# KMASAHIRO/AVR

Hardware: AMD Instinct MI355X
Metric: ray-samples/sec/GPU (1024 rays×256 samp×512 freq) + IR render ms/pose (higher is better)
Workload: dtype f32; 1 GPU; c2_meshrir_1024x256x512; mode=pose, rays=1024, samples=256, T=1022, freq_bins=512, distinct_poses=16, parallelism=poses x1 (no data-path collective)

## Files before the change

avr_amd/_lib.py:

```python
from __future__ import annotations

import ctypes
import math
import os
import threading

import numpy as np
import torch

_HERE = os.path.dirname(os.path.abspath(__file__))
LIB_PATH = os.path.join(_HERE, "libavr_hip.so")

DTYPE_F32 = 0
DTYPE_F16 = 1
DTYPE_BF16 = 2
MAX_AZI = 512
IRFFT_MAX_N = 13476

_c_i32 = ctypes.c_int32
_c_i64 = ctypes.c_int64
_c_f32 = ctypes.c_float
_vp = ctypes.c_void_p


# ... 19 lines not shown
        ("pl_len", _c_i32),
    ]

    def key(self):
        k = self.__dict__.get("_key")
        if k is None:
            k = self._key = tuple(getattr(self, f) for f, _ in self._fields_)
        return k


def _f32(x) -> float:
    return float(np.float32(x))


def render_params(cfg: dict, T: int, n_rays: int | None = None) -> RenderParams:
    p = RenderParams()
    p.n_azi = int(cfg["n_azi"])
    p.n_ele = int(cfg["n_ele"])
    p.n_samples = int(cfg["n_samples"])
    p.T = int(T)
    p.n_rays = p.n_azi * p.n_ele + 2 if n_rays is None else int(n_rays)
    p.depth_scale = _f32(cfg["far"] - cfg["near"])
    p.depth_offset = _f32(cfg["near"])
    p.lo = _f32(cfg["xyz_min"])
    p.span = _f32(cfg["xyz_max"] - cfg["xyz_min"])
    p.fs = _f32(cfg["fs"])
    p.speed = _f32(cfg["speed"])
    p.pathloss = _f32(cfg["pathloss"])
    p.azi_jitter = _f32(np.pi * 2 / cfg["n_azi"])
    p.two_pi = _f32(np.pi * 2)
    p.phase_c = _f32((-2 * np.pi) / T)
    p.near_clamp = int(0.1 / cfg["speed"] * cfg["fs"])
    p.pl_len = int(math.ceil(T * 2.5))
    return p


class TablePtrs(ctypes.Structure):

    _fields_ = [("d_vals", ctypes.c_void_p), ("shift", ctypes.c_void_p),
                ("pl_table", ctypes.c_void_p), ("phase", ctypes.c_void_p),
                ("twiddle", ctypes.c_void_p), ("ir_twiddle", ctypes.c_void_p)]


_SIGS = {
    "avr_last_error": (ctypes.c_char_p, []),
    "avr_abi_version": (ctypes.c_int, []),
    "avr_pinned_alloc": (ctypes.c_int, [_c_i64, _vp, _vp]),
    "avr_pinned_free": (ctypes.c_int, [_vp]),
    "avr_graph_launch": (ctypes.c_int, [_vp, _vp]),
    "avr_tables": (ctypes.c_int, [_vp, _vp, _vp, _vp, _vp, _vp, _vp, _vp]),
    "avr_depth_samples": (ctypes.c_int, [_vp, _vp, _vp]),
    "avr_ir_twiddle": (ctypes.c_int, [_c_i32, _vp, _vp]),
    "avr_ray_directions": (ctypes.c_int, [_vp, _vp, _vp, _vp]),
    "avr_sample_points": (ctypes.c_int, [_vp, _c_i32] + [_vp] * 10),
    "avr_sample_rays": (ctypes.c_int, [_vp, _c_i32, _vp, _c_i32] + [_vp] * 9),
    "avr_weights_fwd": (ctypes.c_int, [_vp, _c_i32, _vp, _c_i32] + [_vp] * 7),
    "avr_ray_reduce_fwd": (ctypes.c_int, [_vp, _c_i32, _vp, _c_i32, _vp, _vp, _c_i32, _vp, _vp]),
    "avr_sample_rays_dev": (ctypes.c_int, [_vp, _c_i32, _vp, _c_i32] + [_vp] * 9),
    "avr_sample_rays_staged": (ctypes.c_int, [_vp, _c_i32, _vp, _c_i32, _c_i32] + [_vp] * 7),
    "avr_reduce_splits": (ctypes.c_int, [_vp, _c_i32, _c_i32, _vp]),
    "avr_ray_reduce_mc_fwd": (ctypes.c_int, [_vp, _c_i32, _c_i32, _vp, _c_i32, _vp, _vp, _vp, _c_i64, _c_i32,
                                             _vp, _vp]),
    "avr_reduce_mc_splits": (ctypes.c_int, [_vp, _c_i32, _c_i32, _c_i32, _vp, _vp]),
    "avr_ray_reduce_mc16_fwd": (ctypes.c_int, [_vp, _c_i32, _c_i32, _vp, _c_i32, _vp, _vp, _vp, _c_i64, _c_i32,
                                               _vp, _vp]),
    "avr_reduce_mc16_max_rays": (_c_i32, []),
    "avr_sh_decode_fwd": (ctypes.c_int, [_c_i32, _c_i32, _c_i32, _c_i32, _vp, _vp, _vp, _vp]),
    "avr_sh_decode_bwd": (ctypes.c_int, [_c_i32, _c_i32, _c_i32, _c_i32, _vp, _vp, _vp, _vp]),
    "avr_ray_reduce_mc_bwd": (ctypes.c_int, [_vp, _c_i32, _c_i32, _vp, _c_i32, _vp, _vp, _vp, _vp, _c_i64,
                                             _vp, _vp, _vp]),
    "avr_dft_phase_fwd": (ctypes.c_int, [_vp, _c_i32, _vp, _c_i32, _vp, _vp, _vp, _vp, _c_i32, _vp, _vp]),
    "avr_spectrum_finalize": (ctypes.c_int, [_c_i32, _c_i32, _c_i32, _vp, _vp, _vp]),
    "avr_irfft": (ctypes.c_int, [_c_i32, _c_i32, _vp, _vp, _vp, _vp]),
    "avr_irfft_bwd": (ctypes.c_int, [_c_i32, _c_i32, _vp, _vp, _vp, _vp]),
    "avr_dft_phase_bwd": (ctypes.c_int, [_vp, _c_i32] + [_vp] * 7),
    "avr_ray_reduce_bwd": (ctypes.c_int, [_vp, _c_i32, _vp, _c_i32] + [_vp] * 6),
    "avr_weights_bwd": (ctypes.c_int, [_vp, _c_i32, _vp, _c_i32, _vp, _vp, _vp, _vp]),
    "avr_hashgrid_fwd": (ctypes.c_int, [_c_i64, _c_i32, _vp, _vp, _c_i32, _vp, _vp, _vp, _vp, _c_i32, _vp]),
    "avr_hashgrid_fwd_lm": (ctypes.c_int, [_c_i64, _c_i32, _vp, _vp, _c_i32, _vp, _vp, _vp, _vp, _c_i32, _vp]),
    "avr_hashgrid_fwd_lm_unit": (ctypes.c_int, [_c_i64, _c_i32, _vp, _vp, _c_i32, _vp, _vp, _vp, _vp, _c_i32, _vp]),
    "avr_ray_pose_bias": (ctypes.c_int, [_c_i32, _c_i32, _c_i32, _vp, _vp, _c_i32, _vp, _vp, _vp, _vp,
                                         _c_i32, _vp, _vp, _vp, _vp, _c_i32, _c_i32, _c_i32, _vp, _vp,
                                         _c_i32, _vp, _vp]),
    "avr_hashgrid_bwd": (ctypes.c_int, [_c_i64, _c_i32, _vp, _vp, _c_i32, _vp, _vp, _vp, _vp, _vp]),
    "avr_hashgrid_bwd_workspace": (ctypes.c_int, [_c_i64, _c_i32, _vp, _vp]),
    "avr_hashgrid_bwd_partitioned": (ctypes.c_int, [_c_i64, _c_i32, _vp, _vp, _c_i32, _vp, _vp, _vp, _vp, _vp,
                                                    _c_i64, _vp]),
    "avr_hashgrid_bwd_partitioned_set": (ctypes.c_int, [_c_i64, _c_i32, _vp, _vp, _c_i32, _vp, _vp, _vp, _vp, _vp,
                                                    _c_i64, _vp]),
    "avr_hashgrid_bwd_input_workspace": (ctypes.c_int, [_c_i64, _c_i32, _vp]),
    "avr_hashgrid_bwd_input": (ctypes.c_int, [_c_i64, _c_i32, _vp, _vp, _c_i32, _vp, _c_i32, _vp, _vp, _vp, _vp, _vp,
                                              _c_i64, _vp]),
    "avr_linear_wgrad_splits": (ctypes.c_int, [_c_i64, _c_i32, _c_i32, _vp]),
    "avr_linear512_pack_w2": (ctypes.c_int, [_vp, _c_i32, _c_i32, _vp, _vp]),
    "avr_linear512_mask_fwd": (ctypes.c_int, [_c_i64, _vp, _vp, _c_i32, _vp, _vp, _vp]),
    "avr_linear_wgrad": (ctypes.c_int, [_c_i64, _c_i32, _c_i32, _vp, _vp, _vp, _c_i32, _vp, _vp]),
    "avr_linear_out1_fwd": (ctypes.c_int, [_c_i64, _c_i32, _vp, _vp, _c_i32, _vp, _vp]),
    "avr_narrow_mm": (ctypes.c_int, [_c_i64, _c_i32, _c_i32, _vp, _vp, _c_i32, _c_i32, _vp, _vp, _vp]),
    "avr_linear_out1_workspace": (ctypes.c_int, [_c_i32, _vp]),
    "avr_linear_out1_bwd": (ctypes.c_int, [_c_i64, _c_i32, _vp, _vp, _vp, _c_i32, _vp, _vp, _vp, _vp]),
    "avr_head_splits": (ctypes.c_int, [_vp, _c_i32, _c_i32, _c_i32, _vp]),
    "avr_head_sort": (ctypes.c_int, [_vp, _c_i32, _vp, _vp, _vp, _vp, _vp, _vp]),
    "avr_head_pack_w": (ctypes.c_int, [_vp, _c_i32, _c_i32, _vp, _c_i32, _vp, _vp]),
    "avr_head_exact_layout": (ctypes.c_int, [_vp, _c_i32, _c_i32, _c_i32, _vp, _vp]),
    "avr_head_pack_w_exact": (ctypes.c_int, [_vp, _c_i32, _vp, _c_i32, _vp, _vp]),
    "avr_head_fwd_exact": (ctypes.c_int, [_vp, _c_i32, _c_i32, _vp, _vp, _c_i32, _vp, _vp, _vp, _vp, _c_i32,
                                          _vp, _vp, _vp]),
    "avr_head_fwd": (ctypes.c_int, [_vp, _c_i32, _c_i32, _vp, _vp, _c_i32, _vp, _vp, _vp, _c_i32, _vp,
                                    _vp]),
    "avr_head_bwd_workspace": (ctypes.c_int, [_vp, _c_i32, _c_i32, _c_i32, _vp]),
    "avr_head_bwd": (ctypes.c_int, [_vp, _c_i32, _c_i32, _vp, _vp, _c_i32, _vp, _vp, _vp, _vp, _vp, _vp,
                                    _vp, _vp, _vp, _vp, _c_i64, _vp]),
    "avr_head_bwd2": (ctypes.c_int, [_vp, _c_i32, _c_i32, _vp, _vp, _c_i32, _vp, _vp, _vp, _vp, _vp, _vp,
                                     _c_i32, _vp, _vp, _vp, _vp, _c_i64, _vp]),
    "avr_criterion_window_len": (ctypes.c_int, []),
    "avr_criterion_workspace": (ctypes.c_int, [_c_i32, _c_i32, _vp]),
    "avr_criterion_fwd": (ctypes.c_int, [_c_i32, _c_i32] + [_vp] * 10 + [_c_i64, _vp]),
    "avr_criterion_fwd2": (ctypes.c_int, [_c_i32, _c_i32] + [_vp] * 11 + [_c_i64, _vp]),
    "avr_criterion_bwd": (ctypes.c_int, [_c_i32, _c_i32] + [_vp] * 11 + [_c_i64, _vp, _vp]),
    "avr_das_workspace": (ctypes.c_int, [_vp]),
    "avr_das_fwd": (ctypes.c_int, [_c_i32] + [_vp] * 5 + [_c_f32] * 3 + [_vp, _vp, _c_i64, _vp]),
    "avr_das_bwd": (ctypes.c_int, [_c_i32] + [_vp] * 3 + [_c_f32] * 3 + [_vp, _vp, _c_i64, _vp, _vp]),
    "avr_metrics_workspace": (ctypes.c_int, [_c_i32, _c_i32, _vp]),
    "avr_metrics": (ctypes.c_int, [_c_i32, _c_i32, ctypes.c_double, _c_i32, _c_i32] + [_vp] * 10
                    + [_c_i64, _vp]),
    "avr_scale_sanitize": (ctypes.c_int, [_c_i32, _vp, _vp, _vp, _vp]),
    "avr_grad_clip_workspace": (ctypes.c_int, [_c_i32, _vp, _vp]),
    "avr_grad_clip_coef": (ctypes.c_int, [_c_i32, _vp, _vp, ctypes.c_float, _vp, ctypes.c_int64, _vp, _vp, _vp]),
    "avr_adam_step": (ctypes.c_int, [_c_i32, _vp, _vp, _vp, _vp, _vp, _vp, _vp, ctypes.c_double, ctypes.c_double,
                                     ctypes.c_float, ctypes.c_float, _vp, _vp]),
    "avr_concat_fwd": (ctypes.c_int, [_c_i64, _c_i32, _vp, _vp, _c_i32, _vp]),
    "avr_concat_bwd": (ctypes.c_int, [_c_i64, _c_i32, _vp, _vp, _c_i32, _vp, _vp]),
    "avr_group_bias_relu_fwd": (ctypes.c_int, [_c_i64, _c_i32, _c_i64, _c_i32, _vp, _c_i32, _vp, _vp, _vp, _vp]),
    "avr_group_bias_relu_workspace": (ctypes.c_int, [_c_i64, _c_i32, _c_i64, _vp]),
    "avr_group_bias_relu_bwd": (ctypes.c_int, [_c_i64, _c_i32, _c_i64, _c_i32, _vp, _vp, _c_i32, _vp, _vp, _vp,
                                               _c_i64, _vp, _vp]),
    "avr_conv_source": (ctypes.c_int, [_c_i32, _c_i32, _c_i32, _c_i64, _vp, _vp, _vp, _vp]),
    "avr_conv_trajectory": (ctypes.c_int, [_c_i32, _c_i32, _c_i32, _c_i64, _c_i64, _c_i64, _vp, _vp, _vp, _vp]),
    "avr_sosfiltfilt_workspace": (ctypes.c_int, [_c_i64, _c_i64, _c_i32, _c_i32, _vp]),
    "avr_sosfiltfilt": (ctypes.c_int, [_c_i64, _c_i64, _c_i32, _c_i32, _vp, _vp, _vp, _c_i32, _vp, _c_i32,
                                       _vp, _c_i64, _vp]),
    "avr_doa_das_workspace": (ctypes.c_int, [_c_i64, _c_i32, _c_i32, _vp]),
    "avr_doa_das": (ctypes.c_int, [_c_i64, _c_i32, _c_i32, _c_i32, _vp, _vp, _vp, _vp, _vp, ctypes.c_double,
                                   _vp, _vp, _c_i32, _vp, _vp, _c_i64, _vp]),
    "avr_doa_frames": (ctypes.c_int, [_c_i64, _c_i64, _c_i32, _c_i32, _c_i64, _c_i32, _c_i32, _c_i32, _c_i32,
                                      _c_i32, _c_f32, _vp, _c_i32, _vp, _vp, _vp, _vp, _vp, _vp, _vp]),
    "avr_doa_frame_stats": (ctypes.c_int, [_c_i64, _c_i64, _vp, _vp, _vp, _vp, _vp, _vp]),
    "avr_sigma_pack_bytes": (ctypes.c_int, [_c_i32, _vp]),
    "avr_sigma_desc_size": (ctypes.c_int, []),
    "avr_sigma_fwd": (ctypes.c_int, [_vp] * 3 + [_c_i32, _vp, _vp]),
    "avr_render_core_layout": (ctypes.c_int, [_vp, _c_i32, _c_i32, _vp, _vp]),
    "avr_render_core_fwd": (ctypes.c_int, [_vp, _c_i32, _vp, _c_i32, _vp, _c_i32] + [_vp] * 5
                            + [_c_i64] + [_vp] * 5),
}

EXPORTS = tuple(_SIGS)

_SHAPES_SIGS = {
    "avr_linear512_pack_w": (ctypes.c_int, [_vp, _c_i32, _vp, _vp]),
    "avr_linear512_relu_fwd": (ctypes.c_int, [_c_i64, _vp, _vp, _c_i32, _vp, _vp]),
    "avr_mlp512x2_pack_w": (ctypes.c_int, [_vp, _vp, _c_i32, _vp, _vp]),
    "avr_mlp512x2_fwd": (ctypes.c_int, [_c_i64, _vp, _vp, _c_i32, _vp, _vp]),
    "avr_linear_pack_w": (ctypes.c_int, [_c_i32, _c_i32, _vp, _c_i32, _vp, _vp]),
}

_lock = threading.Lock()
_lib = None


def load():
    global _lib
    if _lib is not None:
        return _lib
    with _lock:
        if _lib is not None:
            return _lib
        if not os.path.exists(LIB_PATH):
            raise RuntimeError(
                f"avr_amd: HIP library not found at {LIB_PATH}; build it with "
                "`python -c 'import __graft_entry__ as g; g.build()'` (make -C avr_amd/csrc)")
        lib = ctypes.CDLL(LIB_PATH)
        for name, (res, args) in _SIGS.items():
            fn = getattr(lib, name)
            fn.restype = res
            fn.argtypes = args
        for name, (res, args) in _SHAPES_SIGS.items():
            if hasattr(lib, name):
                fn = getattr(lib, name)
                fn.restype = res
                fn.argtypes = args
# ... 21 lines not shown
```

avr_amd/csrc/common.h:

```cpp
#pragma once

#include <hip/hip_runtime.h>
#include <hip/hip_fp16.h>
#include <hip/hip_bf16.h>
#include <type_traits>
#include <stdint.h>
#include <string>
#include <utility>

#include "avr_hip.h"

namespace avr {

void set_error(const std::string& msg);
int fail(int code, const std::string& msg);
int check_launch(const char* what);
int device_cus();

#define AVR_REQUIRE(cond, msg)                          \
    do {                                                \
        if (!(cond)) return ::avr::fail(AVR_E_ARG, msg); \
    } while (0)

int validate_render_params(const avr_render_params* p);

int launch_irfft(int B, int F, const float* spec, const float* spec2, const float* tw, float* ir,
                 float* ir2, void* stream);
constexpr int kIrfftMaxN = AVR_IRFFT_MAX_N;
constexpr size_t kLdsPerCu = 160 * 1024;
#define AVR_IRFFT_LIMIT_TEXT "irfft length n > 13476 not supported (n*12 B of twiddles and data must fit the 160 KiB LDS)"

int mr3_workspace(int B, int n, int64_t* bytes);
int launch_mr3(int B, int n, const float* pred_time, const float* ori_time, const float* wtab,
               const float* tw512, void* ws, int64_t ws_bytes, float* out, void* stream);

inline hipStream_t as_stream(void* s) { return reinterpret_cast<hipStream_t>(s); }

constexpr size_t kLdsDefault = 64 * 1024;

template <typename Kern, typename... Args>
int launch(const char* what, Kern kern, dim3 grid, dim3 block, size_t lds, hipStream_t st,
           Args&&... args) {
    if (lds > kLdsPerCu)
        return fail(AVR_E_CONFIG, std::string(what) + ": " + std::to_string(lds) +
                                      " B of dynamic LDS exceed a CU's 160 KiB");
    if (lds > kLdsDefault) {
        const hipError_t e = hipFuncSetAttribute((const void*)kern,
                                                 hipFuncAttributeMaxDynamicSharedMemorySize, (int)lds);
        if (e != hipSuccess)
            return fail((int)e, std::string(what) + ": LDS opt-in: " + hipGetErrorString(e));
    }
    hipLaunchKernelGGL(kern, grid, block, lds, st, std::forward<Args>(args)...);
    return check_launch(what);
}

constexpr int64_t align_up(int64_t x, int64_t a) { return (x + a - 1) & ~(a - 1); }

class Arena {
  public:
    Arena(void* base, int64_t align) : base_(static_cast<char*>(base)), align_(align) {}
    template <typename T>
    T* take(int64_t count) {
        char* r = base_ ? base_ + off_ : nullptr;
        off_ += align_up(count * (int64_t)sizeof(T), align_);
        return reinterpret_cast<T*>(r);
    }
    int64_t offset() const { return off_; }
    int64_t bytes() const { return off_; }

  private:
    char* base_;
    int64_t align_, off_ = 0;
};

template <int Code>
struct dtype_tag;
template <>
struct dtype_tag<AVR_DTYPE_F32> { using type = float; };
template <>
struct dtype_tag<AVR_DTYPE_F16> { using type = __half; };
template <>
struct dtype_tag<AVR_DTYPE_BF16> { using type = __hip_bfloat16; };

template <int... Allowed, typename F>
int dispatch_dtype(int code, const char* what, F&& f) {
    int rc = 0;
    const bool hit = ((code == Allowed ? (rc = f(dtype_tag<Allowed>{}), true) : false) || ...);
    return hit ? rc : fail(AVR_E_ARG, std::string(what) + ": unsupported dtype");
}

__device__ __forceinline__ void mfma_queue_wait() {
    __builtin_amdgcn_sched_barrier(0);
    asm volatile("s_nop 7");
}
template <typename T>
__device__ __forceinline__ void keep_live(const T& v) {
    asm volatile("" ::"v"(v));
}

__device__ __forceinline__ float load_f(const float* p, int64_t i) { return p[i]; }
__device__ __forceinline__ float load_f(const __half* p, int64_t i) { return __half2float(p[i]); }
__device__ __forceinline__ float load_f(const __hip_bfloat16* p, int64_t i) {
    return __bfloat162float(p[i]);
}
__device__ __forceinline__ void store_f(float* p, int64_t i, float v) { p[i] = v; }
__device__ __forceinline__ void store_f(__half* p, int64_t i, float v) { p[i] = __float2half(v); }
__device__ __forceinline__ void store_f(__hip_bfloat16* p, int64_t i, float v) {
    p[i] = __float2bfloat16(v);
}
__device__ __forceinline__ float bf16_lo(uint32_t u) { return __uint_as_float(u << 16); }
__device__ __forceinline__ float bf16_hi(uint32_t u) { return __uint_as_float(u & 0xffff0000u); }
__device__ __forceinline__ float f16_lo(uint32_t u) { return __half2float(__ushort_as_half((unsigned short)(u & 0xffffu))); }
__device__ __forceinline__ float f16_hi(uint32_t u) { return __half2float(__ushort_as_half((unsigned short)(u >> 16))); }

template <typename T>
__device__ __forceinline__ float unpack16(uint32_t u, int hi) {
    if constexpr (std::is_same<T, __half>::value)
        return hi ? f16_hi(u) : f16_lo(u);
    else
// ... 167 lines not shown
```

avr_amd/csrc/hashgrid.hip:

```cpp
#include "common.h"

#include <algorithm>

using namespace avr;

namespace {

constexpr int kMaxLevels = 32;

struct LevelTable {
    int64_t offset[kMaxLevels + 1];
    float scale[kMaxLevels];
    uint32_t res[kMaxLevels];
};

__device__ __forceinline__ uint32_t grid_index(uint32_t size, uint32_t res, uint32_t x, uint32_t y,
                                               uint32_t z) {
    uint64_t stride = 1;
    uint32_t index = 0;
    const uint32_t c[3] = {x, y, z};
#pragma unroll
    for (int d = 0; d < 3; ++d) {
        if (stride > size) break;
        index += c[d] * (uint32_t)stride;
// ... 101 lines not shown
            w *= 1.0f - c.pos[d];
            g[d] = c.grid[d];
        }
    }
    e = grid_index(size, res, g[0], g[1], g[2]);
}

__device__ __forceinline__ void corner_dx(const Corner& c, int k, uint32_t size, uint32_t res, float (&dw)[3],
                                          uint32_t& e) {
    float om[3];
    uint32_t g[3];
#pragma unroll
    for (int d = 0; d < 3; ++d) {
        const bool up = k & (1 << d);
        om[d] = up ? c.pos[d] : 1.0f - c.pos[d];
        g[d] = up ? c.grid[d] + 1 : c.grid[d];
    }
    const float w12 = om[1] * om[2], w02 = om[0] * om[2], w01 = om[0] * om[1];
    dw[0] = (k & 1) ? w12 : -w12;
    dw[1] = (k & 2) ? w02 : -w02;
    dw[2] = (k & 4) ? w01 : -w01;
    e = grid_index(size, res, g[0], g[1], g[2]);
}

template <typename Tp>
__device__ __forceinline__ float2 encode_point_level(const float* xi, const Level<const Tp>& lv) {
    const Corner c = locate(xi, lv.scale);
    CornerAcc<Tp> acc;
#pragma unroll
    for (int k = 0; k < 8; ++k) {
        float w;
        uint32_t e;
        corner(c, k, lv.size, lv.res, w, e);
        acc.add(w, CornerAcc<Tp>::load(lv.table, e));
    }
    return acc.get();
}

template <typename Tp, typename To>
__global__ __launch_bounds__(256) void hashgrid_fwd_kernel(int64_t N, int L,
                                                           const float* __restrict__ x,
                                                           const Tp* __restrict__ params,
                                                           LevelTable lt, To* __restrict__ out) {
    const int64_t q = (int64_t)blockIdx.x * blockDim.x + threadIdx.x;
    if (q >= N * L) return;
    const int64_t i = q / L;
    const int l = (int)(q % L);
    const float xi[3] = {x[i * 3 + 0], x[i * 3 + 1], x[i * 3 + 2]};
    const Level<const Tp> lv = level_view(lt, l, params);
    const Corner c = locate(xi, lv.scale);
    CornerAcc<Tp> acc;
#pragma unroll
    for (int k = 0; k < 8; ++k) {
        float w;
        uint32_t e;
        corner(c, k, lv.size, lv.res, w, e);
        acc.add(w, CornerAcc<Tp>::load(lv.table, e));
    }
    store_pair(out, q, acc.get());
}

template <typename Tp>
struct EntryGroup;
template <>
struct EntryGroup<__half> {
    static constexpr uint32_t kN = 4;
    uint32_t d[4];
    __device__ __forceinline__ void load(const __half* table, uint32_t e) {
        const uint4 v = *reinterpret_cast<const uint4*>(table + 2 * (e & ~(kN - 1)));
        d[0] = v.x;
        d[1] = v.y;
        d[2] = v.z;
        d[3] = v.w;
    }
    __device__ __forceinline__ __half2 get(uint32_t e) const {
        const uint32_t j = e & (kN - 1);
        const uint32_t v = j == 0 ? d[0] : j == 1 ? d[1] : j == 2 ? d[2] : d[3];
        __half2 h;
        __builtin_memcpy(&h, &v, 4);
        return h;
    }
};

template <typename Tp, typename To, bool ROW_MAJOR = false, bool GROUP = false>
__global__ __launch_bounds__(256) void hashgrid_fwd_lm_kernel(int64_t N, const float* __restrict__ x,
                                                              const Tp* __restrict__ params,
                                                              LevelTable lt, To* __restrict__ out, int unit) {
    const int l = blockIdx.y;
    const int64_t i = (int64_t)blockIdx.x * 256 + threadIdx.x;
    if (i >= N) return;
    float xi[3] = {x[i * 3 + 0], x[i * 3 + 1], x[i * 3 + 2]};
    if (unit) {
#pragma unroll
        for (int d = 0; d < 3; ++d) xi[d] = 0.5f + 0.5f * xi[d];
    }
    const Level<const Tp> lv = level_view(lt, l, params);
    const Tp* table = lv.table;
    const Corner c = locate(xi, lv.scale);
    CornerAcc<Tp> acc;
    float wgt[8];
    uint32_t ent[8];
#pragma unroll
    for (int k = 0; k < 8; ++k) corner(c, k, lv.size, lv.res, wgt[k], ent[k]);
    if constexpr (GROUP) {
        constexpr uint32_t kN = EntryGroup<Tp>::kN;
        EntryGroup<Tp> grp[4];
#pragma unroll
        for (int j = 0; j < 4; ++j) grp[j].load(table, ent[2 * j]);
        using raw = typename CornerAcc<Tp>::raw;
        raw far[4];
#pragma unroll
        for (int j = 0; j < 4; ++j) {
            far[j] = grp[j].get(ent[2 * j]);
            if ((ent[2 * j + 1] ^ ent[2 * j]) >= kN) far[j] = CornerAcc<Tp>::load(table, ent[2 * j + 1]);
        }
#pragma unroll
        for (int j = 0; j < 4; ++j) {
            const raw v0 = grp[j].get(ent[2 * j]);
            const raw v1 = ((ent[2 * j + 1] ^ ent[2 * j]) >= kN) ? far[j] : grp[j].get(ent[2 * j + 1]);
            acc.add(wgt[2 * j], v0);
            acc.add(wgt[2 * j + 1], v1);
        }
    } else {
#pragma unroll
        for (int k = 0; k < 8; ++k) acc.add(wgt[k], CornerAcc<Tp>::load(table, ent[k]));
    }
    store_pair(out, ROW_MAJOR ? i * (int64_t)gridDim.y + l : (int64_t)l * N + i, acc.get());
}

template <typename Tp, typename Tg>
__global__ __launch_bounds__(256) void hashgrid_dx_level_kernel(int64_t N, const float* __restrict__ x,
                                                                const Tp* __restrict__ params,
                                                                const Tg* __restrict__ gout, LevelTable lt,
                                                                float* __restrict__ partial) {
    const int l = blockIdx.y, L = gridDim.y;
    const int64_t i = (int64_t)blockIdx.x * 256 + threadIdx.x;
    if (i >= N) return;
    const float xi[3] = {x[i * 3 + 0], x[i * 3 + 1], x[i * 3 + 2]};
    const float g0 = load_f(gout, i * (2 * L) + 2 * l), g1 = load_f(gout, i * (2 * L) + 2 * l + 1);
    const Level<const Tp> lv = level_view(lt, l, params);
    const Corner c = locate(xi, lv.scale);
    float dw[8][3];
    uint32_t ent[8];
#pragma unroll
    for (int k = 0; k < 8; ++k) corner_dx(c, k, lv.size, lv.res, dw[k], ent[k]);
    float2 v[8];
#pragma unroll
    for (int k = 0; k < 8; ++k) v[k] = load_pair<Tp>(lv.table, ent[k]);
    float acc[3] = {0.0f, 0.0f, 0.0f};
#pragma unroll
    for (int k = 0; k < 8; ++k) {
        const float t = fmaf(g1, v[k].y, g0 * v[k].x);
#pragma unroll
        for (int d = 0; d < 3; ++d) acc[d] = fmaf(dw[k][d], t, acc[d]);
    }
    float* p = partial + ((int64_t)l * N + i) * 3;
#pragma unroll
    for (int d = 0; d < 3; ++d) p[d] = lv.scale * acc[d];
}

__global__ __launch_bounds__(256) void hashgrid_dx_sum_kernel(int64_t M, int L, const float* __restrict__ partial,
                                                              float* __restrict__ grad_x) {
    const int64_t j = (int64_t)blockIdx.x * 256 + threadIdx.x;
    if (j >= M) return;
    float s = 0.0f;
    for (int l = 0; l < L; ++l) s += partial[(int64_t)l * M + j];
    grad_x[j] = s;
}

template <typename Tg, int RUN>
__global__ __launch_bounds__(256) void hashgrid_bwd_kernel(int64_t N, int L, int l0,
                                                           const float* __restrict__ x,
                                                           const Tg* __restrict__ gout,
                                                           LevelTable lt,
                                                           float* __restrict__ gparams) {
    const int l = l0 + (int)blockIdx.y;
    const int slot = threadIdx.x & 15;
    const int k = slot >> 1, f = slot & 1;
    const int64_t first = ((int64_t)blockIdx.x * 16 + (threadIdx.x >> 4)) * RUN;
    const Level<float> lv = level_view(lt, l, gparams);
    float* __restrict__ table = lv.table;
    float xi[RUN][3], g[RUN];
#pragma unroll
    for (int it = 0; it < RUN; ++it) {
        const int64_t i = first + it;
        const int64_t ic = i < N ? i : N - 1;
#pragma unroll
        for (int d = 0; d < 3; ++d) xi[it][d] = x[ic * 3 + d];
        g[it] = i < N ? load_f(gout, ic * (2 * L) + 2 * l + f) : 0.0f;
    }
    uint32_t pe = 0xffffffffu;
    float pv = 0.0f;
#pragma unroll
    for (int it = 0; it < RUN; ++it) {
        float wgt;
        uint32_t ce;
        corner(locate(xi[it], lv.scale), k, lv.size, lv.res, wgt, ce);
        const uint32_t e = 2u * ce + (uint32_t)f;
        const float v = wgt * g[it];
        if (e == pe) {
            pv += v;
        } else {
            if (pv != 0.0f) atomicAdd(table + pe, pv);
            pe = e;
            pv = v;
        }
    }
    if (pv != 0.0f) atomicAdd(table + pe, pv);
}

// ... 580 lines not shown
                  0);
}

extern "C" int avr_hashgrid_fwd_lm_unit(int64_t N, int32_t n_levels, const float* x, const void* params,
                                        int32_t param_dtype, const int64_t* level_offset,
                                        const float* level_scale, const int32_t* level_res, void* out,
                                        int32_t out_dtype, void* stream) {
    return fwd_lm(N, n_levels, x, params, param_dtype, level_offset, level_scale, level_res, out, out_dtype, stream,
                  1);
}

namespace {

constexpr int kBiasRays = 4;

__device__ __forceinline__ float round_feature(float v, bool f16, bool mlp_f16) {
    if (f16) v = __half2float(__float2half(v));
    return mlp_f16 ? __half2float(__float2half(v))
                   : __bfloat162float(__float2bfloat16(v));
}

template <typename Tp>
__device__ __forceinline__ void bias_features(bool is_tx, int64_t b, int64_t r, int R, int S, const float* view,
                                              const float* tx, const Tp* dp, const LevelTable& dl, const Tp* tp,
                                              const LevelTable& tl, int l, int f16, int mlp_f16, float* e) {
    const float* src = is_tx ? tx + b * R * S * 3 : view + (b * R * S + r * S) * 3;
    const float xi[3] = {(src[0] + 1.0f) / 2.0f, (src[1] + 1.0f) / 2.0f, (src[2] + 1.0f) / 2.0f};
    const float2 v = is_tx ? encode_point_level(xi, level_view(tl, l, tp)) : encode_point_level(xi, level_view(dl, l, dp));
    e[2 * l] = round_feature(v.x, f16, mlp_f16);
    e[2 * l + 1] = round_feature(v.y, f16, mlp_f16);
}

template <typename Tp>
__global__ __launch_bounds__(256) void ray_pose_bias_kernel(int B, int R, int S, const float* __restrict__ view,
                                                            const float* __restrict__ tx, const Tp* __restrict__ dp,
                                                            LevelTable dl, int dL, const Tp* __restrict__ tp,
                                                            LevelTable tl, int tL, int f16, int mlp_f16,
                                                            const float* __restrict__ wd,
                                                            const float* __restrict__ wt, int nout,
                                                            float* __restrict__ bias) {
    __shared__ float e[kBiasRays][2][2 * kMaxLevels];
    const int64_t g0 = (int64_t)blockIdx.x * kBiasRays;
    const int nr = (int)min((int64_t)kBiasRays, (int64_t)B * R - g0);
    for (int q = threadIdx.x; q < kBiasRays * 2 * kMaxLevels; q += 256) {
        const int j = q / (2 * kMaxLevels), rem = q % (2 * kMaxLevels);
        const int which = rem / kMaxLevels, l = rem % kMaxLevels;
        if (j >= nr || l >= (which ? tL : dL)) continue;
        const int64_t gr = g0 + j;
        bias_features(which, gr / R, gr % R, R, S, view, tx, dp, dl, tp, tl, l, f16, mlp_f16, e[j][which]);
    }
    __syncthreads();
    auto skinny = [&](const float* __restrict__ w, int K2, int which, int o, float (&acc)[kBiasRays]) {
        int k = 0;
        for (; k + 8 <= K2; k += 8) {
            float wv[8];
#pragma unroll
            for (int u = 0; u < 8; ++u) wv[u] = w[(int64_t)(k + u) * nout + o];
#pragma unroll
            for (int u = 0; u < 8; ++u)
#pragma unroll
                for (int j = 0; j < kBiasRays; ++j) acc[j] = fmaf(e[j][which][k + u], wv[u], acc[j]);
        }
        for (; k < K2; ++k) {
            const float wv = w[(int64_t)k * nout + o];
#pragma unroll
            for (int j = 0; j < kBiasRays; ++j) acc[j] = fmaf(e[j][which][k], wv, acc[j]);
        }
    };
    for (int o = threadIdx.x; o < nout; o += 256) {
        float sd[kBiasRays], st[kBiasRays];
#pragma unroll
        for (int j = 0; j < kBiasRays; ++j) sd[j] = st[j] = 0.0f;
        skinny(wd, 2 * dL, 0, o, sd);
        skinny(wt, 2 * tL, 1, o, st);
#pragma unroll
        for (int j = 0; j < kBiasRays; ++j)
            if (j < nr) bias[(g0 + j) * nout + o] = sd[j] + st[j];
    }
}

constexpr int kBias2Rays = 4;
constexpr int kBias2Threads = 512;

template <typename Tp>
__global__ __launch_bounds__(kBias2Threads) void ray_pose_bias2_kernel(
    int B, int R, int S, const float* __restrict__ view, const float* __restrict__ tx, const Tp* __restrict__ dp,
    LevelTable dl, int dL, const Tp* __restrict__ tp, LevelTable tl, int tL, int f16, int mlp_f16,
    const float* __restrict__ wd, const float* __restrict__ wt, int nout, float* __restrict__ bias) {
    __shared__ float ed[kBias2Rays][2 * kMaxLevels];
    __shared__ float et[2 * kMaxLevels];
    const int64_t g0 = (int64_t)blockIdx.x * kBias2Rays;
    const int64_t b = g0 / R;
    for (int q = threadIdx.x; q < (kBias2Rays + 1) * kMaxLevels; q += kBias2Threads) {
        const int j = q / kMaxLevels, l = q % kMaxLevels;
        const bool is_tx = j == kBias2Rays;
        if (l >= (is_tx ? tL : dL)) continue;
        bias_features(is_tx, b, (g0 + j) % R, R, S, view, tx, dp, dl, tp, tl, l, f16, mlp_f16, is_tx ? et : ed[j]);
    }
    __syncthreads();
    for (int o = threadIdx.x; o < nout; o += kBias2Threads) {
        constexpr int KB = 16;
        float st = 0.0f;
        for (int k0 = 0; k0 < 2 * tL; k0 += KB) {
            float w[KB];
#pragma unroll
            for (int u = 0; u < KB; ++u) w[u] = k0 + u < 2 * tL ? wt[(int64_t)(k0 + u) * nout + o] : 0.0f;
#pragma unroll
            for (int u = 0; u < KB; ++u)
                if (k0 + u < 2 * tL) st = fmaf(et[k0 + u], w[u], st);
        }
        float sd[kBias2Rays];
#pragma unroll
        for (int r = 0; r < kBias2Rays; ++r) sd[r] = 0.0f;
        for (int k0 = 0; k0 < 2 * dL; k0 += KB) {
            float w[KB];
#pragma unroll
            for (int u = 0; u < KB; ++u) w[u] = k0 + u < 2 * dL ? wd[(int64_t)(k0 + u) * nout + o] : 0.0f;
#pragma unroll
            for (int u = 0; u < KB; ++u)
                if (k0 + u < 2 * dL)
#pragma unroll
                    for (int r = 0; r < kBias2Rays; ++r) sd[r] = fmaf(ed[r][k0 + u], w[u], sd[r]);
        }
#pragma unroll
        for (int r = 0; r < kBias2Rays; ++r) bias[(g0 + r) * nout + o] = sd[r] + st;
    }
}

}

extern "C" int avr_ray_pose_bias(int32_t B, int32_t R, int32_t S, const float* view, const float* tx,
                                 int32_t dir_levels, const void* dir_params, const int64_t* dir_offset,
                                 const float* dir_scale, const int32_t* dir_res, int32_t tx_levels,
                                 const void* tx_params, const int64_t* tx_offset, const float* tx_scale,
                                 const int32_t* tx_res, int32_t param_dtype, int32_t enc_dtype,
                                 int32_t mlp_dtype, const float* w_dir, const float* w_tx, int32_t n_out,
                                 float* bias, void* stream) {
    AVR_REQUIRE(B >= 1 && R >= 1 && S >= 1 && view && tx && dir_params && tx_params && w_dir && w_tx && bias &&
                    n_out >= 1,
                "avr_ray_pose_bias: bad args");
    AVR_REQUIRE(enc_dtype == AVR_DTYPE_F16 || enc_dtype == AVR_DTYPE_F32, "avr_ray_pose_bias: enc dtype");
    AVR_REQUIRE(mlp_dtype == AVR_DTYPE_BF16 || mlp_dtype == AVR_DTYPE_F16, "avr_ray_pose_bias: mlp dtype");
    const int mlp_f16 = mlp_dtype == AVR_DTYPE_F16;
    LevelTable dl, tl;
    if (int e = make_table(dir_levels, dir_offset, dir_scale, dir_res, &dl)) return e;
    if (int e = make_table(tx_levels, tx_offset, tx_scale, tx_res, &tl)) return e;
    const int64_t rays = (int64_t)B * R;
    const dim3 grid((unsigned)((rays + kBiasRays - 1) / kBiasRays));
    const int f16 = enc_dtype == AVR_DTYPE_F16;
    hipStream_t st = as_stream(stream);
    const bool v2 = R % kBias2Rays == 0;
    return dispatch_dtype<AVR_DTYPE_F16, AVR_DTYPE_F32>(param_dtype, "avr_ray_pose_bias", [&](auto tag) {
        using Tp = typename decltype(tag)::type;
        auto go = [&](auto kern, dim3 g, dim3 block) {
            return launch("avr_ray_pose_bias", kern, g, block, 0, st, (int)B, (int)R, (int)S, view, tx,
                          (const Tp*)dir_params, dl, (int)dir_levels, (const Tp*)tx_params, tl, (int)tx_levels, f16,
                          mlp_f16, w_dir, w_tx, (int)n_out, bias);
        };
        if (v2) return go(ray_pose_bias2_kernel<Tp>, dim3((unsigned)(rays / kBias2Rays)), dim3(kBias2Threads));
        return go(ray_pose_bias_kernel<Tp>, grid, dim3(256));
    });
}

constexpr int64_t kPartitionedMinPoints = 16384;

extern "C" int avr_hashgrid_bwd_workspace(int64_t N, int32_t n_levels, const int64_t* level_offset,
                                          int64_t* bytes) {
    AVR_REQUIRE(N >= 0 && level_offset && bytes, "avr_hashgrid_bwd_workspace: bad args");
    if (N < kPartitionedMinPoints) {
        *bytes = 256;
        return 0;
    }
    if (n_levels < 1 || n_levels > kMaxLevels) return fail(AVR_E_ARG, "hashgrid: n_levels out of range (1..32)");
    BwdLayout b;
    *bytes = (bwd_layout(N, n_levels, level_offset, nullptr, &b) == 0 && b.scatter_ok) ? b.bytes : 256;
    return 0;
}

namespace {
int bwd_partitioned(int64_t N, int32_t n_levels, const float* x, const void* grad_out, int32_t grad_dtype,
                    const int64_t* level_offset, const float* level_scale, const int32_t* level_res,
                    float* grad_params, void* workspace, int64_t workspace_bytes, void* stream, bool overwrite) {
    AVR_REQUIRE(N >= 0 && x && grad_out && level_offset && level_scale && level_res && grad_params && workspace,
                "avr_hashgrid_bwd_partitioned: bad args");
    AVR_REQUIRE(reinterpret_cast<uintptr_t>(grad_params) % 16 == 0 && reinterpret_cast<uintptr_t>(workspace) % 256 == 0,
                "avr_hashgrid_bwd_partitioned: grad_params must be 16-byte, workspace 256-byte aligned");
    AVR_REQUIRE(grad_dtype == AVR_DTYPE_F32 || grad_dtype == AVR_DTYPE_F16,
                "avr_hashgrid_bwd_partitioned: unknown grad dtype");
    LevelTable lt;
    if (int e = make_table(n_levels, level_offset, level_scale, level_res, &lt)) return e;
    hipStream_t st = as_stream(stream);
    const int L = n_levels;
    const char* what = "avr_hashgrid_bwd_partitioned";
    BwdLayout b;
    if (N < kPartitionedMinPoints || bwd_layout(N, n_levels, level_offset, level_res, &b) != 0 || !b.scatter_ok) {
        if (overwrite &&
            hipMemsetAsync(grad_params, 0, (size_t)(2 * level_offset[L]) * sizeof(float), st) != hipSuccess)
            return fail(AVR_E_ARG, "avr_hashgrid_bwd_partitioned_set: clear failed");
        return N == 0 ? 0 : launch_bwd(what, st, N, L, x, grad_out, grad_dtype, lt, grad_params);
    }
    AVR_REQUIRE(workspace_bytes >= b.bytes, "avr_hashgrid_bwd_partitioned: workspace too small");
    char* ws = static_cast<char*>(workspace);
    int* counts = reinterpret_cast<int*>(ws + b.counts);
    int* totals = reinterpret_cast<int*>(ws + b.totals);
    uint3* contrib = reinterpret_cast<uint3*>(ws + b.contrib);
    const dim3 grid((unsigned)b.plan.nchunks, (unsigned)L);
    const size_t lds_count = (size_t)b.plan.max_parts * 4;
    const size_t lds_scat = (size_t)(3 * kScatMaxRecs + 3 * b.plan.max_parts + 1) * 4;
    const dim3 tgrid((unsigned)((N + 63) / 64));
    void* glm = ws + b.glm;
    int* part_start = reinterpret_cast<int*>(ws + b.part_start);
    int* slice_base = reinterpret_cast<int*>(ws + b.slice_base);
    if (int e = dispatch_dtype<AVR_DTYPE_F32, AVR_DTYPE_F16>(grad_dtype, what, [&](auto tag) {
            using Tg = typename decltype(tag)::type;
            const Tg* g = (const Tg*)glm;
            if (int e = launch(what, hg_level_major_kernel<Tg>, tgrid, dim3(256), 64 * 2 * L * sizeof(Tg), st, N, L,
                               (const Tg*)grad_out, (Tg*)glm))
                return e;
            if (int e = launch(what, hg_bwd_count_kernel<Tg>, grid, dim3(256), lds_count, st, N, L, x, g, lt, b.plan,
                               counts))
                return e;
            if (int e = launch(what, hg_bwd_scan_kernel, dim3((unsigned)((b.total_parts + 15) / 16)), dim3(1024), 0,
                               st, b.total_parts, b.plan.nchunks, counts, totals))
                return e;
            if (int e = launch(what, hg_bwd_plan_kernel, dim3(1), dim3(1024), 0, st, b.total_parts, b.plan, totals,
                               part_start, slice_base))
                return e;
            return launch(what, hg_bwd_scatter_kernel<Tg>, grid, dim3(256), lds_scat, st, N, L, x, g, lt, b.plan,
                          counts, totals, part_start, contrib);
        }))
        return e;
    if (overwrite)
        if (int e = launch(what, hg_bwd_zero_hot_kernel, dim3((unsigned)b.total_parts), dim3(256), 0, st, lt, b.plan,
                           b.total_parts, slice_base, grad_params))
            return e;
    return launch(what, hg_bwd_reduce_kernel, dim3((unsigned)((b.max_slices + kReduceWaves - 1) / kReduceWaves)),
                  dim3(64 * kReduceWaves), 0, st, lt, b.plan, b.total_parts, totals, part_start, slice_base, contrib,
                  grad_params, (int)overwrite);
}
}

extern "C" int avr_hashgrid_bwd_partitioned(int64_t N, int32_t n_levels, const float* x, const void* grad_out,
                                            int32_t grad_dtype, const int64_t* level_offset,
// ... 56 lines not shown
```

avr_amd/csrc/head.hip:

```cpp
#include "common.h"

using namespace avr;

namespace {

constexpr int kThreads = 256;

__device__ __forceinline__ void lds_barrier() {
    __builtin_amdgcn_s_waitcnt(0xC07F);
    __builtin_amdgcn_s_barrier();
}

template <typename Th, int KB>
struct Raw {
    static constexpr int NB = KB * (int)sizeof(Th);
    static constexpr int ND = NB / 4;
    uint32_t d[ND];
    __device__ __forceinline__ void load(const Th* p) {
        if constexpr (NB % 16 == 0) {
#pragma unroll
            for (int c = 0; c < NB / 16; ++c) {
                const u32x4 v = reinterpret_cast<const u32x4*>(p)[c];
                d[4 * c] = v[0];
                d[4 * c + 1] = v[1];
// ... 320 lines not shown
        for (int k = 0; k < KB; ++k) run[k] = fmaf(wr[u], hv[u][k], run[k]);
    float off[KB];
#pragma unroll
    for (int k = 0; k < KB; ++k) {
        const float x = wave_scan_incl(run[k]);
        off[k] = dpp<0x138, 0xf, true>(x);
        if (lane == 63) wtotf[wave * KB + k] = x;
    }
    lds_barrier();
#pragma unroll
    for (int k = 0; k < KB; ++k) {
        float o = 0.0f;
        for (int w = 0; w < wave; ++w) o += wtotf[w * KB + k];
        off[k] += o;
    }
    if (threadIdx.x == 0)
#pragma unroll
        for (int k = 0; k < KB; ++k) C[k * RS + 3] = 0.0f;
    if (RPT % 4 == 0 && spt == RPT) {
        if (p0 < n)
#pragma unroll
            for (int k = 0; k < KB; ++k) {
                float r = 0.0f;
#pragma unroll
                for (int c = 0; c < RPT / 4; ++c) {
                    float v[4];
#pragma unroll
                    for (int e = 0; e < 4; ++e) {
                        r = fmaf(wr[4 * c + e], hv[4 * c + e][k], r);
                        v[e] = off[k] + r;
                    }
                    *reinterpret_cast<f32x4*>(C + k * RS + 4 + p0 + 4 * c) = f32x4{v[0], v[1], v[2], v[3]};
                }
            }
    } else {
#pragma unroll
        for (int k = 0; k < KB; ++k) {
            float r = 0.0f;
#pragma unroll
            for (int u = 0; u < RPT; ++u) {
                r = fmaf(wr[u], hv[u][k], r);
                if (u < spt && p0 + u < n) C[k * RS + 4 + p0 + u] = off[k] + r;
            }
        }
    }
}

template <int RPT>
struct Owned {
    int ray[RPT];
    float w[RPT];
    int n, spt;
    __device__ __forceinline__ void load(const int* __restrict__ perm, const float* __restrict__ ws,
                                         const int* __restrict__ cnt, int T) {
        n = cnt[T - 1];
        spt = (n + kThreads - 1) / kThreads;
#pragma unroll
        for (int u = 0; u < RPT; ++u) {
            const int p = threadIdx.x * spt + u;
            const bool ok = u < spt && p < n;
            ray[u] = ok ? perm[p] : 0;
            w[u] = ok ? ws[p] : 0.0f;
        }
    }
};

template <typename Th, int KB, int RPT>
__device__ __forceinline__ void load_sorted_rows(Raw<Th, KB> (&v)[RPT], const Th* __restrict__ h, int64_t hrow0,
                                                 int64_t hstride, int k0, const Owned<RPT>& own) {
#pragma unroll
    for (int u = 0; u < RPT; ++u) v[u].load(h + hrow0 + (int64_t)own.ray[u] * hstride + k0);
}

__host__ __device__ constexpr size_t cumsum_lds_bytes(int R, int KB) {
    return 4 * ((size_t)KB * cs_stride(R) + 4 * (size_t)KB);
}

template <int RPT>
__global__ __launch_bounds__(kThreads) void head_sort_kernel(avr_render_params pp, int R,
                                                             const float* __restrict__ w,
                                                             const int32_t* __restrict__ delay,
                                                             int* __restrict__ perm_out,
                                                             float* __restrict__ ws_out,
                                                             int* __restrict__ cnt_out) {
    extern __shared__ float lds_f[];
    const int T = pp.T, S = pp.n_samples;
    const int s = blockIdx.x, b = blockIdx.y;
    const int nk = pow2_ceil(R);
    int* cnt = reinterpret_cast<int*>(lds_f);
    float* wr = reinterpret_cast<float*>(cnt + T);
    uint32_t* keys = reinterpret_cast<uint32_t*>(wr + R);
    int* wtot = reinterpret_cast<int*>(keys + nk);
    Rays<RPT> rays;
    rays.load(w, delay, b, s, R, S);
    const int n = sort_rays<RPT>(rays, tail_limit(pp, s), T, R, cnt, wr, keys, nk, wtot);
    const int64_t col = (int64_t)b * S + s;
    for (int p = threadIdx.x; p < R; p += kThreads) {
        const int r = p < n ? (int)(keys[p] & 0xfffu) : 0;
        perm_out[col * R + p] = r;
        ws_out[col * R + p] = p < n ? wr[r] : 0.0f;
    }
    for (int t = threadIdx.x; t < T; t += kThreads) cnt_out[col * T + t] = cnt[t];
}

template <typename Th>
__global__ __launch_bounds__(kThreads) void head_pack_w_kernel(int T, int K, int KB, const Th* __restrict__ W,
                                                               Th* __restrict__ Wp) {
    const int64_t n = (int64_t)T * K;
    for (int64_t i = blockIdx.x * (int64_t)kThreads + threadIdx.x; i < n; i += (int64_t)gridDim.x * kThreads) {
        const int j = (int)(i % KB);
        const int64_t r = i / KB;
        const int t = (int)(r % T), kb = (int)(r / T);
        Wp[i] = W[(int64_t)t * K + kb * KB + j];
    }
}

template <typename Th, int KB, int NT, int RPT, int SB>
__global__ __launch_bounds__(kThreads) void head_fwd_kernel(avr_render_params pp, int B, int R, int K,
                                                            int KG, const Th* __restrict__ h,
                                                            const Th* __restrict__ W,
                                                            const int* __restrict__ perm,
                                                            const float* __restrict__ ws,
                                                            const int* __restrict__ cnt,
                                                            float* __restrict__ zpart) {
    extern __shared__ float lds_f[];
    const int T = pp.T, S = pp.n_samples;
    const int kg = blockIdx.x, s = blockIdx.y, b = blockIdx.z;
    float* C = lds_f;
    const int RS = cs_stride(R);
    float* wtotf = C + KB * RS;
    const int lim = tail_limit(pp, s);
    const int64_t col = (int64_t)b * S + s;
    const int64_t hrow0 = ((int64_t)b * R * S + s) * K;
    const int64_t hstride = (int64_t)S * K;
    const int kbeg = kg * KG, kend = kbeg + KG;
    Raw<Th, KB> wt[NT];
    load_wpacked<Th, KB, NT>(wt, W, kbeg, T);
    Owned<RPT> own;
    own.load(perm + col * R, ws + col * R, cnt + col * T, T);
    int ct[NT];
#pragma unroll
    for (int i = 0; i < NT; ++i) ct[i] = cnt[col * T + min((int)threadIdx.x + kThreads * i, T - 1)];
    float zacc[NT];
#pragma unroll
    for (int i = 0; i < NT; ++i) zacc[i] = 0.0f;
    auto contract = [&](int k0) {
#pragma unroll
        for (int i = 0; i < NT; ++i) {
            const int t = threadIdx.x + kThreads * i;
            if (t < lim) {
                float a = zacc[i];
#pragma unroll
                for (int k = 0; k < KB; ++k) a = fmaf(wt[i][k], C[k * RS + 3 + ct[i]], a);
                zacc[i] = a;
            }
        }
        if (k0 + KB < kend) load_wpacked<Th, KB, NT>(wt, W, k0 + KB, T);
        lds_barrier();
    };
    if constexpr (SB == 1) {
        Raw<Th, KB> hv[RPT];
        load_sorted_rows<Th, KB, RPT>(hv, h, hrow0, hstride, kbeg, own);
        for (int k0 = kbeg; k0 < kend; k0 += KB) {
            build_cumsum<Th, KB, RPT>(C, R, own.n, own.spt, own.w, hv, wtotf);
            if (k0 + KB < kend) load_sorted_rows<Th, KB, RPT>(hv, h, hrow0, hstride, k0 + KB, own);
            lds_barrier();
            contract(k0);
        }
    } else {
        constexpr int ND = Raw<Th, KB>::ND;
// ... 405 lines not shown
        lds_sort > 150 * 1024)
        return fail(AVR_E_CONFIG, "fused head: T x rays too large for LDS");
    if (K % kb != 0 || (kb * es) % 8 != 0)
        return fail(AVR_E_CONFIG, "fused head: hidden width must be a multiple of the feature block");
    int n = 1;
    const int64_t cols = (int64_t)B * S;
    while (n < 16 && cols * n < 1024 && (K / (2 * n)) % kb == 0 && K % (2 * n) == 0) n *= 2;
    hs->rpt = R <= 4 * kThreads ? 4 : (R <= 8 * kThreads ? 8 : 16);
    hs->nt = nt;
    hs->kb = kb;
    hs->n_kg = n;
    hs->kg = K / n;
    hs->lds_q = (size_t)kb * q_stride(T) * 4;
    hs->lds_c = cumsum_lds_bytes(R, kb);
    hs->lds_sort = lds_sort;
    return 0;
}

int elem_size(int dtype) { return dtype == AVR_DTYPE_F32 ? 4 : 2; }

int head_check(const avr_render_params* p, int B, int K, const void* h, const void* W, int dtype) {
    AVR_REQUIRE(p && B >= 1 && K >= 4 && h && W, "fused head: bad args");
    AVR_REQUIRE(dtype == AVR_DTYPE_F32 || dtype == AVR_DTYPE_BF16 || dtype == AVR_DTYPE_F16,
                "fused head: h/W must be fp32, bf16 or fp16");
    AVR_REQUIRE(reinterpret_cast<uintptr_t>(h) % 16 == 0 && reinterpret_cast<uintptr_t>(W) % 16 == 0,
                "fused head: h and W must be 16-byte aligned");
    return 0;
}

#ifndef AVR_HEAD_DW_TARGET
#define AVR_HEAD_DW_TARGET 512
#endif
void dw_groups(const HeadShape& hs, int B, int S, int K, int* n_sg, int* s_per) {
    const int nkb = K / hs.kb;
    int n = 1;
    while (n < S && (int64_t)nkb * n * B < AVR_HEAD_DW_TARGET) n *= 2;
    *s_per = (S + n - 1) / n;
    *n_sg = (S + *s_per - 1) / *s_per;
}

void fwd_block(const HeadShape& hs, int dtype, int* kb, int* sb) {
    int kbf = hs.kb, s = 1;
    if (elem_size(dtype) == 2 && hs.rpt <= 8) {
        kbf = hs.kb > 8 ? 8 : hs.kb;
        s = hs.nt <= 4 ? 4 : 2;
        if (hs.kg % (s * kbf) != 0) s = 1;
    }
    *kb = kbf;
    *sb = s;
}

int pack_w(const char* what, int T, int K, int kb, const void* W, int dtype, void* Wp, hipStream_t st) {
    const int64_t n = (int64_t)T * K;
    const int blocks = (int)std::min<int64_t>((n + kThreads - 1) / kThreads, 4096);
    return dispatch_dtype<AVR_DTYPE_BF16, AVR_DTYPE_F16, AVR_DTYPE_F32>(dtype, what, [&](auto tag) {
        using TH = typename decltype(tag)::type;
        return launch(what, head_pack_w_kernel<TH>, dim3(blocks), dim3(kThreads), 0, st, T, K, kb, (const TH*)W,
                      (TH*)Wp);
    });
}

}

extern "C" int avr_head_pack_w(const avr_render_params* p, int32_t B, int32_t K, const void* W, int32_t dtype,
                               void* Wp, void* stream) {
    if (int e = head_check(p, B, K, W, W, dtype)) return e;
    AVR_REQUIRE(Wp && reinterpret_cast<uintptr_t>(Wp) % 16 == 0, "avr_head_pack_w: Wp must be 16-byte aligned");
    HeadShape hs;
    if (int e = head_shape(*p, B, n_rays(*p), K, elem_size(dtype), &hs)) return e;
    int kbf, sb;
    fwd_block(hs, dtype, &kbf, &sb);
    return pack_w("avr_head_pack_w", p->T, K, kbf, W, dtype, Wp, as_stream(stream));
}

extern "C" int avr_head_splits(const avr_render_params* p, int32_t B, int32_t K, int32_t dtype,
                               int32_t* n_split) {
    AVR_REQUIRE(p && n_split, "avr_head_splits: bad args");
    HeadShape hs;
    if (int e = head_shape(*p, B, n_rays(*p), K, elem_size(dtype), &hs)) return e;
    *n_split = hs.n_kg;
    return 0;
}

extern "C" int avr_head_sort(const avr_render_params* p, int32_t B, const float* w, const int32_t* delay,
                             int32_t* perm, float* ws, int32_t* cnt, void* stream) {
    AVR_REQUIRE(p && B >= 1 && w && delay && perm && ws && cnt, "avr_head_sort: bad args");
    const int R = n_rays(*p);
    HeadShape hs;
    if (int e = head_shape(*p, B, R, 16, 4, &hs)) return e;
    hipStream_t st = as_stream(stream);
    const dim3 grid(p->n_samples, B);
    auto kern = hs.rpt == 4 ? head_sort_kernel<4> : hs.rpt == 8 ? head_sort_kernel<8> : head_sort_kernel<16>;
    return launch("avr_head_sort", kern, grid, dim3(kThreads), hs.lds_sort, st, *p, R, w, delay, perm, ws, cnt);
}

extern "C" int avr_head_fwd(const avr_render_params* p, int32_t B, int32_t K, const void* h,
                            const void* W, int32_t dtype, const int32_t* perm, const float* ws,
                            const int32_t* cnt, int32_t n_split, float* zpart, void* stream) {
    if (int e = head_check(p, B, K, h, W, dtype)) return e;
    AVR_REQUIRE(perm && ws && cnt && zpart, "avr_head_fwd: bad args");
    const int R = n_rays(*p);
    HeadShape hs;
    if (int e = head_shape(*p, B, R, K, elem_size(dtype), &hs)) return e;
    hipStream_t st = as_stream(stream);
    int kbf, sb;
    fwd_block(hs, dtype, &kbf, &sb);
    AVR_REQUIRE(n_split == hs.n_kg, "avr_head_fwd: n_split must come from avr_head_splits");
    const dim3 grid(hs.n_kg, p->n_samples, B);
    HeadShape hf = hs;
    hf.kb = kbf;
    hf.lds_c = cumsum_lds_bytes(R, kbf);
#define AVR_HF(KBV, NTV, RP)                                                                       \
    if (hf.kb == KBV && hf.nt == NTV && hf.rpt == RP) {                                            \
        constexpr bool kSb = sizeof(TH) == 2 && RP <= 8;                                            \
        if (kSb && sb == 2) return go(head_fwd_kernel<TH, KBV, NTV, RP, kSb ? 2 : 1>);              \
        if (kSb && sb == 4) return go(head_fwd_kernel<TH, KBV, NTV, RP, kSb ? 4 : 1>);              \
        return go(head_fwd_kernel<TH, KBV, NTV, RP, 1>);                                            \
    }
#define AVR_HF_R(KBV, NTV) AVR_HF(KBV, NTV, 4) AVR_HF(KBV, NTV, 8) AVR_HF(KBV, NTV, 16)
    return dispatch_dtype<AVR_DTYPE_BF16, AVR_DTYPE_F16, AVR_DTYPE_F32>(dtype, "avr_head_fwd", [&](auto tag) {
        using TH = typename decltype(tag)::type;
        auto go = [&](auto kern) {
            return launch("avr_head_fwd", kern, grid, dim3(kThreads), hf.lds_c, st, *p, (int)B, R, (int)K, hf.kg,
                          (const TH*)h, (const TH*)W, perm, ws, cnt, zpart);
        };
        AVR_HF_R(4, 4) AVR_HF_R(4, 8) AVR_HF_R(4, 16) AVR_HF_R(8, 4) AVR_HF_R(8, 8) AVR_HF_R(16, 4)
        return fail(AVR_E_CONFIG, "avr_head_fwd: no kernel for this block shape");
    });
#undef AVR_HF_R
#undef AVR_HF
}

bool hb_blk_ok(int B, int S, int K) { return K % 8 == 0 && (int64_t)B * S <= 65535; }
int hb_parts(const HeadShape& hs, int B, int S, int K) {
    return hb_blk_ok(B, S, K) ? std::max(hs.n_kg, (K + kHbFeat - 1) / kHbFeat) : hs.n_kg;
}
int64_t hb_sum_floats(int B, int S, int T, int K) {
    return hb_blk_ok(B, S, K) ? (int64_t)B * S * (hb_nblk(T) + 2 * hb_nseg(T)) * K : 0;
}

extern "C" int avr_head_bwd_workspace(const avr_render_params* p, int32_t B, int32_t K, int32_t dtype,
                                      int64_t* bytes) {
    AVR_REQUIRE(p && bytes, "avr_head_bwd_workspace: bad args");
    const int R = n_rays(*p), S = p->n_samples, T = p->T;
    HeadShape hs;
    if (int e = head_shape(*p, B, R, K, elem_size(dtype), &hs)) return e;
    int n_sg, s_per;
    dw_groups(hs, B, S, K, &n_sg, &s_per);
    *bytes = ((int64_t)hb_parts(hs, B, S, K) * B * R * S + (int64_t)B * n_sg * T * K) * 4 + 16 +
             (int64_t)T * K * (elem_size(dtype)) + hb_sum_floats(B, S, T, K) * 4 + 16;
    return 0;
}

extern "C" int avr_head_bwd(const avr_render_params* p, int32_t B, int32_t K, const void* h,
                            const void* W, int32_t dtype, const float* w, const int32_t* delay,
                            const int32_t* perm, const float* ws, const int32_t* cnt, const float* gz,
                            void* grad_h, float* grad_w, float* grad_W, float* workspace,
                            int64_t workspace_bytes, void* stream) {
    return avr_head_bwd2(p, B, K, h, W, dtype, w, delay, perm, ws, cnt, gz, 0, grad_h, grad_w, grad_W, workspace,
                         workspace_bytes, stream);
}

extern "C" int avr_head_bwd2(const avr_render_params* p, int32_t B, int32_t K, const void* h,
                             const void* W, int32_t dtype, const float* w, const int32_t* delay,
                             const int32_t* perm, const float* ws, const int32_t* cnt, const float* gz,
                             int32_t relu_mask, void* grad_h, float* grad_w, float* grad_W, float* workspace,
                             int64_t workspace_bytes, void* stream) {
    if (int e = head_check(p, B, K, h, W, dtype)) return e;
    AVR_REQUIRE(relu_mask == 0 || relu_mask == 1, "avr_head_bwd: relu_mask must be 0 or 1");
    AVR_REQUIRE(w && delay && perm && ws && cnt && gz && grad_h && grad_w && grad_W && workspace,
                "avr_head_bwd: bad args");
    const int R = n_rays(*p), S = p->n_samples, T = p->T;
    HeadShape hs;
    if (int e = head_shape(*p, B, R, K, elem_size(dtype), &hs)) return e;
    int n_sg, s_per;
    dw_groups(hs, B, S, K, &n_sg, &s_per);
// ... 69 lines not shown
```

avr_amd/csrc/head_exact.hip:

```cpp
#include "common.h"
#include "mma.h"
#include "probe.h"
#include "stationary.h"

#include <algorithm>

using namespace avr;

AVR_PROBE_TU(avr_probe_set_exact)

namespace {

constexpr int kExactMaxT[2] = {4096, 1024};

__host__ __device__ constexpr int xs_tile_bytes(int KSM) { return KSM * 1024; }
constexpr int kPartBufs = 2;
constexpr int kReadAhead = 8;
constexpr int kHold = 4;

__host__ __device__ constexpr size_t xs_lds_bytes(int KSM, int T, int waves, int rays, int nb, int nc) {
    return (size_t)nb * nc * xs_tile_bytes(KSM) + 4 * (size_t)((T + 3) / 4 * 4) + 4 * (size_t)rays +
           4 * (size_t)(kPartBufs * waves * 32 * nc) + 4 * (size_t)waves + 8;
}

// ... 222 lines not shown
                if (half == 0) zr[buf * (WAVES * TT) + wave * TT + 32 * c + j] = v;
            };
            auto sum_tile = [&](int tau, int buf) {
                if (lane < TT) {
                    const float* zz = zr + buf * (WAVES * TT) + lane;
                    float v = zz[0];
#pragma unroll
                    for (int w = 1; w < WAVES; ++w) v += zz[TT * w];
                    const int t = TT * tau + lane;
                    if (t < T) zc[t] = v;
                }
            };
            auto summer = [&](int m) { return m % WAVES; };
            for (int tau = tb; tau < te; ++tau) {
                const int i = tau - tb;
                AVR_PROBE_BEGIN(comp);
                const int dtile = tau + NB - 1 < te ? tau + NB - 1 : -1;
                const int dslot = (i + NB - 1) % NB;
                bool issued = false;
                float zl[NC];
#pragma unroll
                for (int c = 0; c < NC; ++c) {
                    const int t0 = TT * tau + 32 * c;
                    zl[c] = 0.0f;
                    if (t0 + 31 >= dstart[wave] && t0 < lim) {
                        const f32x16 acc = chain(i % NB, c, issued ? -1 : dtile, dslot);
                        issued = true;
                        zl[c] = epi(acc, tau, c);
                    }
                }
                if (dtile >= 0 && !issued) issue(dtile, dslot);
                AVR_PROBE_END(comp, 6);
#pragma unroll
                for (int c = 0; c < NC; ++c) put(zl[c], i % kPartBufs, c);
                AVR_PROBE_BEGIN(dma);
                if (tau + 1 < te) {
                    int st = 0;
                    for (int m = max(0, i + 2 - NB); m < i; ++m) st += (wave == summer(m));
                    wait_vm(min(NB - 2, te - 2 - tau) * DPW + st);
                }
                if (i == min(1, te - 1 - tb)) {
                    load_dly(nx);
                    dly_issued = true;
                }
                if (tau == te - 1) {
                    touch(nx);
                    touched = true;
                }
                AVR_PROBE_END(dma, 4);
                AVR_PROBE_BEGIN(bar);
                lgkmcnt0();
                __builtin_amdgcn_s_barrier();
                AVR_PROBE_END(bar, 5);
                if (wave == summer(i)) sum_tile(tau, i % kPartBufs);
            }
            for (int t = tid; t < T; t += NT)
                if (t < TT * tb || t >= TT * te) zc[t] = 0.0f;
        }
        if (!dly_issued) load_dly(nx);
        if (!touched) touch(nx);
        if (tid == 0 && !published) qnext[iter & 1] = item_of(3 * gq + claim);
        if (p0 >= nk || lim <= 0) __syncthreads();
        AVR_PROBE_FLUSH((int64_t)item * WAVES + wave);
        item = nxt;
        nxt = qnext[(iter + 1) & 1];
        cur = nx;
    }
}

__global__ __launch_bounds__(256) void head_pack_exact_kernel(int T, int K, int KSM, const uint16_t* __restrict__ W,
                                                              frag8* __restrict__ Wf, int64_t n) {
    for (int64_t i = blockIdx.x * (int64_t)256 + threadIdx.x; i < n; i += (int64_t)gridDim.x * 256) {
        const int lane = (int)(i & 63);
        const int64_t r = i >> 6;
        const int ks = (int)(r % KSM);
        const int tau = (int)(r / KSM);
        const int t = 32 * tau + (lane & 31), k0 = 16 * ks + 8 * (lane >> 5);
        frag8 v = frag8{0u, 0u, 0u, 0u};
        if (t < T && k0 < K) v = *reinterpret_cast<const frag8*>(W + (int64_t)t * K + k0);
        Wf[i] = v;
    }
}

constexpr int kExactQueueInts = 256;

int exact_ksm(int K) { return K <= 128 ? 8 : (K <= 256 ? 16 : 32); }

struct ExactShape {
    int rays;
    bool tt64;
};

ExactShape exact_shape(int R, int T, int K) {
    ExactShape sh{(R <= 16 * 128 && T <= 1024) ? 128 : 256, false};
    if (K == 512) sh = {256, true};
    if (const char* e = AVR_PROBE_ENV("AVR_EXACT_RAYS_PROBE")) sh.rays = atoi(e) == 256 ? 256 : 128;
    if (const char* e = AVR_PROBE_ENV("AVR_EXACT_TT_PROBE")) sh.tt64 = atoi(e) == 64;
    if (sh.rays == 128 || K != 512) sh.tt64 = false;
    return sh;
}

int exact_check(const avr_render_params* p, int32_t K, int32_t dtype) {
    AVR_REQUIRE(p, "avr_head_fwd_exact: bad args");
    AVR_REQUIRE(dtype == AVR_DTYPE_F16 || dtype == AVR_DTYPE_BF16, "avr_head_fwd_exact: h/W must be fp16 or bf16");
    if (K % 16 != 0 || K < 16 || K > 512) return fail(AVR_E_CONFIG, "exact head: K must be a multiple of 16, <= 512");
    const int R = n_rays(*p);
    AVR_REQUIRE(R >= 1 && R <= 16 * 256 && p->T >= 2 && p->T <= 4096 && p->n_samples >= 1,
                "avr_head_fwd_exact: shape out of range (<= 4096 rays per shard, T <= 4096)");
    return 0;
}

size_t exact_lds(int R, int T, int K) {
    const int KSM = exact_ksm(K);
    const ExactShape sh = exact_shape(R, T, K);
    if (sh.rays == 128) return xs_lds_bytes(KSM, T, 4, 128, 2, 1);
    if (sh.tt64) return xs_lds_bytes(KSM, T, 8, 256, 2, 2);
    return xs_lds_bytes(KSM, T, 8, 256, 4, 1);
}

int exact_splits(int R, int T, int K) {
    const int rays = exact_shape(R, T, K).rays;
    const int nb = (R + rays - 1) / rays;
    int n = 1;
    while (n < nb) n *= 2;
    return n;
}

}

extern "C" int avr_head_exact_layout(const avr_render_params* p, int32_t B, int32_t K, int32_t dtype,
                                     int32_t* n_split, int64_t* wpack_bytes) {
    AVR_REQUIRE(B >= 1 && n_split && wpack_bytes, "avr_head_exact_layout: bad args");
    if (int e = exact_check(p, K, dtype)) return e;
    if (exact_lds(n_rays(*p), p->T, K) > 160 * 1024)
        return fail(AVR_E_CONFIG, "exact head: LDS image above 160 KiB for this shape");
    *n_split = exact_splits(n_rays(*p), p->T, K);
    *wpack_bytes = (int64_t)((p->T + 63) / 64) * 2 * xs_tile_bytes(exact_ksm(K));
    return 0;
}

extern "C" int avr_head_pack_w_exact(const avr_render_params* p, int32_t K, const void* W, int32_t dtype,
                                     void* Wf, void* stream) {
    AVR_REQUIRE(W && Wf, "avr_head_pack_w_exact: bad args");
    if (int e = exact_check(p, K, dtype)) return e;
    AVR_REQUIRE(reinterpret_cast<uintptr_t>(W) % 16 == 0 && reinterpret_cast<uintptr_t>(Wf) % 16 == 0,
                "avr_head_pack_w_exact: W and Wf must be 16-byte aligned");
    const int T = p->T, KSM = exact_ksm(K);
    const int64_t n = (int64_t)((T + 63) / 64) * 2 * KSM * 64;
    const int blocks = (int)std::min<int64_t>((n + 255) / 256, 4096);
    return launch("avr_head_pack_w_exact", head_pack_exact_kernel, dim3(blocks), dim3(256), 0,
                  as_stream(stream), T, (int)K, KSM, (const uint16_t*)W, (frag8*)Wf, n);
}

extern "C" int avr_head_fwd_exact(const avr_render_params* p, int32_t B, int32_t K, const void* h, const void* Wf,
                                  int32_t dtype, const int32_t* perm, const float* ws, const int32_t* cnt,
                                  const int32_t* delay, int32_t n_split, float* zpart, int32_t* queue,
                                  void* stream) {
    AVR_REQUIRE(p && B >= 1 && h && Wf && perm && ws && cnt && delay && zpart && queue,
                "avr_head_fwd_exact: bad args");
    if (int e = exact_check(p, K, dtype)) return e;
    AVR_REQUIRE(reinterpret_cast<uintptr_t>(h) % 16 == 0 && reinterpret_cast<uintptr_t>(Wf) % 16 == 0,
                "avr_head_fwd_exact: h and Wf must be 16-byte aligned");
    const int R = n_rays(*p), S = p->n_samples, T = p->T;
    AVR_REQUIRE(n_split == exact_splits(R, T, K), "avr_head_fwd_exact: n_split must be avr_head_exact_layout's");
    if (exact_lds(R, T, K) > 160 * 1024)
        return fail(AVR_E_CONFIG, "exact head: LDS image above 160 KiB for this shape");
    const int64_t items = (int64_t)n_split * B * S;
    AVR_REQUIRE(items < (1ll << 31), "avr_head_fwd_exact: too many columns");
    const int KSM = exact_ksm(K);
    hipStream_t st = as_stream(stream);
    const ExactShape shape = exact_shape(R, T, K);
    const bool small = shape.rays == 128, tt64 = shape.tt64;
    int prio = small ? 0 : 1;
    if (const char* pe = AVR_PROBE_ENV("AVR_EXACT_PRIO_PROBE")) prio = atoi(pe);
    return dispatch_dtype<AVR_DTYPE_F16, AVR_DTYPE_BF16>(dtype, "avr_head_fwd_exact", [&](auto e_tag) {
        using E = typename decltype(e_tag)::type;
        auto go = [&](auto kern, int ksm, int waves, int rays, int nb, int nc, const void* hv) {
            const size_t lds = xs_lds_bytes(ksm, T, waves, rays, nb, nc);
            int per_cu = 1;
            if (hipOccupancyMaxActiveBlocksPerMultiprocessor(&per_cu, kern, 64 * waves, lds) != hipSuccess ||
                per_cu < 1)
                per_cu = 1;
            const int64_t gq = std::min<int64_t>((int64_t)device_cus() * per_cu / 8, (items + 7) / 8);
            const int grid = 8 * (int)std::max<int64_t>(gq, 1);
            (void)hipMemsetAsync(queue, 0, kExactQueueInts * sizeof(int32_t), st);
            return launch("avr_head_fwd_exact", kern, dim3(grid), dim3(64 * waves), lds, st, *p, (int)B, R, (int)K,
                          (const E*)hv, (const frag8*)Wf, perm, ws, cnt, delay, zpart, (int*)queue, (int)items, prio);
        };
        const bool rowdma = K == 512;
        if (small) {
            if (KSM == 8) return go(head_exact_kernel<E, 8, 4, 128, 2, 1, false>, 8, 4, 128, 2, 1, h);
            if (KSM == 16) return go(head_exact_kernel<E, 16, 4, 128, 2, 1, false>, 16, 4, 128, 2, 1, h);
            if (rowdma) return go(head_exact_kernel<E, 32, 4, 128, 2, 1, true>, 32, 4, 128, 2, 1, h);
            return go(head_exact_kernel<E, 32, 4, 128, 2, 1, false>, 32, 4, 128, 2, 1, h);
        }
        if (tt64 && rowdma) return go(head_exact_kernel<E, 32, 8, 256, 2, 2, true>, 32, 8, 256, 2, 2, h);
        if (KSM == 8) return go(head_exact_kernel<E, 8, 8, 256, 4, 1, false>, 8, 8, 256, 4, 1, h);
        if (KSM == 16) return go(head_exact_kernel<E, 16, 8, 256, 4, 1, false>, 16, 8, 256, 4, 1, h);
        if (rowdma) return go(head_exact_kernel<E, 32, 8, 256, 4, 1, true>, 32, 8, 256, 4, 1, h);
        return go(head_exact_kernel<E, 32, 8, 256, 4, 1, false>, 32, 8, 256, 4, 1, h);
    });
}
```

avr_amd/model.py:

```python
from __future__ import annotations

import math

import torch
import torch.nn as nn
import torch.nn.functional as F

import os

from . import sigma as _sigma
from .chembed import group_bias_relu
from .concat import grouped_concat
from .encoding import HashGridEncoding
from .options import DEFAULT, KernelOptions, resolve
from .wcache import cache_lookup, cache_store, capturing, cast_weight

_WGRAD_ROWS = 4096


def _wgrad_hip(gy, x):
    import ctypes

    from . import _lib

# ... 375 lines not shown
    def hidden(self, x, ch=None, rows_per_group=None, link=None):
        if ch is None:
            return MLP._chain(self, x, list(self.hidden_layers), link)
        if rows_per_group is None:
            rows_per_group = x.size(0) // ch.numel()
        ch = ch.reshape(-1).to(device=x.device, dtype=torch.int64)
        x = x.to(self.dtype).contiguous()
        cache = not torch.is_grad_enabled()
        for lin, emb in zip(self.hidden_layers, self.layer_embeddings):
            y = _Linear.apply(x, lin.weight, self.dtype, cache, self.options)
            x = group_bias_relu(y, emb, ch, rows_per_group, self.options)
        return x

    last = MLP.last

    def forward(self, x, ch=None, rows_per_group=None):
        return self.last(self.hidden(x, ch, rows_per_group))


class _Broadcast(torch.autograd.Function):

    @staticmethod
    def forward(ctx, e, view_shape, shape):
        ctx.view_shape = view_shape
        return e.view(view_shape).expand(shape).contiguous()

    @staticmethod
    def backward(ctx, g):
        dims = tuple(i for i, n in enumerate(ctx.view_shape) if n == 1)
        gs = g.sum(dim=dims, keepdim=True, dtype=torch.float32)
        return gs.to(g.dtype).view(-1, g.size(-1)), None, None


def _grouped(enc, x, layout, per):
    if layout is None:
        return enc(x)
    B, R, S = layout
    if per == "sample":
        return enc(x).view(B, R, S, -1)
    if per == "ray":
        e = enc(x.view(B, R, S, 3)[:, :, 0].reshape(B * R, 3))
        return _Broadcast.apply(e, (B, R, 1, e.size(-1)), (B, R, S, e.size(-1)))
    e = enc(x.view(B, R * S, 3)[:, 0].contiguous())
    return _Broadcast.apply(e, (B, 1, 1, e.size(-1)), (B, R, S, e.size(-1)))


def _fused_sigma_ok(model, pts, layout, variant):
    return (layout is not None and pts.is_cuda and not torch.is_grad_enabled()
            and model.options.fused_sigma and _sigma.variant_of(model) == variant)


def _concat_ok(pts, layout, opts=DEFAULT):
    return layout is not None and pts.is_cuda and opts.grouped_concat


_HALF = torch.tensor(0.5)


def _unit(x):
    return torch.add(_HALF, x, alpha=0.5)


def _per_ray(x, layout):
    B, R, S = layout
    return x.reshape(B, R, S, 3)[:, :, 0].reshape(B * R, 3)


def _per_pose(x, layout):
    B, R, S = layout
    return x.reshape(B, R * S, 3)[:, 0].contiguous()


def _bias_columns(w1, dtype=torch.bfloat16):
    key = (w1.data_ptr(), w1._version, dtype)
    hit = None if capturing() else cache_lookup(w1, "_avr_bias_cols", key)
    if hit is not None:
        return hit
    wb = cast_weight(w1, dtype, True).float()
    cols = (wb[:, 128:168].t().contiguous(), wb[:, 168:208].t().contiguous())
    return cols if capturing() else cache_store(w1, "_avr_bias_cols", key, cols)


def _ray_pose_bias(dir_enc, tx_enc, view, tx, wd, wt, layout, mlp_dtype=torch.bfloat16):
    B, R, S = layout
    if not (view.is_cuda and dir_enc.dtype == tx_enc.dtype and dir_enc.param_dtype == tx_enc.param_dtype
            and dir_enc.n_levels <= 32 and tx_enc.n_levels <= 32
            and wd.size(0) == dir_enc.n_output_dims and wt.size(0) == tx_enc.n_output_dims):
        return None
    from . import _lib
    from .encoding import _code
    v = view.reshape(B, R * S, 3).float().contiguous()
    t = tx.reshape(B, R * S, 3).float().contiguous()
    cache = not torch.is_grad_enabled()
    dtab, ttab = dir_enc.table(cache), tx_enc.table(cache)
    bias = torch.empty(B * R, wd.size(1), dtype=torch.float32, device=view.device)
    st = torch.cuda.current_stream(view.device).cuda_stream
    _lib.call("avr_ray_pose_bias", B, R, S, v.data_ptr(), t.data_ptr(),
              dir_enc.n_levels, dtab.data_ptr(), *dir_enc.level_meta(),
              tx_enc.n_levels, ttab.data_ptr(), *tx_enc.level_meta(), _code(dtab.dtype), _code(dir_enc.dtype),
              _lib.DTYPE_F16 if mlp_dtype == torch.float16 else _lib.DTYPE_BF16,
              wd.data_ptr(), wt.data_ptr(), wd.size(1), bias.data_ptr(), st)
    return bias


def _sigma_params(model):
    return _sigma.network_layers(model._model_encoder_sigma) + _sigma.network_layers(model._model_decoder_sigma)


def _cat_features(parts, layout):
    if layout is None:
        return torch.cat(parts, -1)
    return torch.cat(parts, -1).view(-1, sum(p.size(-1) for p in parts))


def _embed_rows(table, ch, n):
    return table[ch].unsqueeze(1).expand(-1, n, -1).reshape(ch.numel() * n, table.size(1))


class AVRModel(nn.Module):

    def __init__(self, cfg, mlp_dtype=torch.float32, enc_dtype=torch.float16, options=None):
        super().__init__()
        o = self.options = resolve(options)
        self._pos_encoding = HashGridEncoding(3, cfg["pos_encoding_sigma"], dtype=enc_dtype, seed=1, options=o)
        self._dir_encoding = HashGridEncoding(3, cfg["dir_encoding_sig"], dtype=enc_dtype, seed=2, options=o)
        self._tx_encoding = HashGridEncoding(3, cfg["tx_encoding_sig"], dtype=enc_dtype, seed=3, options=o)
        self.signal_output_dim = int(cfg["signal_output_dim"])

        ch = cfg.get("channel_embed") or {}
        is_embed = bool(ch.get("is_embed", False))
        conn = ch.get("connection_type", None)
        self.ch_num = int(ch.get("ch_num", 0))
        dims = {"enc": int(ch.get("emb_dim_sigma_encoder", 0)), "dec": int(ch.get("emb_dim_sigma_decoder", 0)),
                "sig": int(ch.get("emb_dim_signal_network", 0))}
        flags = {"enc": bool(ch.get("is_sigma_encoder", False)), "dec": bool(ch.get("is_sigma_decoder", False)),
                 "sig": bool(ch.get("is_signal_network", False))}
        self.enc_injection, self.dec_injection, self.sig_injection = (
            is_embed and conn == "add" and flags[k] for k in ("enc", "dec", "sig"))
        self.enc_concat, self.dec_concat, self.sig_concat = (
            is_embed and conn == "concat" and flags[k] for k in ("enc", "dec", "sig"))
        self.emb_dim_enc, self.emb_dim_dec, self.emb_dim_sig = dims["enc"], dims["dec"], dims["sig"]

        def network(n_in, n_out, net_cfg, inject, concat, emb_name, emb_dim):
            if inject:
                return InjectionMLP(n_in, n_out, net_cfg, self.ch_num, mlp_dtype, o)
            if concat:
                setattr(self, emb_name, nn.Parameter(
                    torch.randn(self.ch_num, emb_dim) / (math.sqrt(emb_dim) if emb_dim else 1.0)))
                n_in += emb_dim
            return MLP(n_in, n_out, net_cfg, mlp_dtype, o)

        self._model_encoder_sigma = network(self._pos_encoding.n_output_dims, 128, cfg["sigma_encoder_network"],
                                            self.enc_injection, self.enc_concat, "encoder_channel_embedding",
                                            self.emb_dim_enc)
        self._model_decoder_sigma = network(128, 1, cfg["sigma_decoder_network"], self.dec_injection,
                                            self.dec_concat, "decoder_channel_embedding", self.emb_dim_dec)
        sig_in = 128 + self._dir_encoding.n_output_dims + self._tx_encoding.n_output_dims
        self._model_signal = network(sig_in, self.signal_output_dim, cfg["signal_network"], self.sig_injection,
                                     self.sig_concat, "signal_channel_embedding", self.emb_dim_sig)
        self.encoder_mode, self.decoder_mode, self.signal_mode = (
            "injection" if i else "concat" if c else "none"
            for i, c in ((self.enc_injection, self.enc_concat), (self.dec_injection, self.dec_concat),
                         (self.sig_injection, self.sig_concat)))
        self._has_embed = (self.encoder_mode, self.decoder_mode, self.signal_mode) != ("none",) * 3
        self._sigma_pack = _sigma.SigmaWeights()

    accepts_ray_layout = True
    supports_fused_head = True
    draws_no_device_rng = True

    def _channel(self, pts, ch_idx):
        if not self._has_embed:
            return None
        if ch_idx is None:
            if "concat" in (self.encoder_mode, self.decoder_mode, self.signal_mode):
                raise ValueError("AVRModel: a 'concat' channel embedding needs ch_idx (its networks' inputs "
                                 "include the embedding row)")
            return None
        ch = torch.as_tensor(ch_idx, device=pts.device).reshape(-1).to(torch.int64)
        if ch.numel() != pts.size(0):
            raise ValueError(f"AVRModel: ch_idx has {ch.numel()} entries for a batch of {pts.size(0)}")
        return ch

    @staticmethod
    def _append_embedding(x, table, ch, n, L, dtype, grouped):
        E = table.size(1)
        if grouped and E >= 8 and E % 8 == 0 and x.size(1) % 8 == 0 and x.size(1) + E <= 512:
            return grouped_concat([(x, 1), (table[ch], n)], x.size(0), dtype, splits=[1, L[1]])
        return torch.cat([x.to(dtype), _embed_rows(table, ch, n).to(dtype)], -1)

    def _trunk(self, pts, view, tx, ch_idx, ray_layout):
        ch = self._channel(pts, ch_idx)
        bs, n = pts.size(0), pts.size(1)
        N = bs * n
        L = ray_layout
        if not self._has_embed and _fused_sigma_ok(self, pts, L, _sigma.MESHRIR):
            return self._trunk_fused(pts, view, tx, L)
        grouped = _concat_ok(pts, L, self.options)
        enc, dec = self._model_encoder_sigma, self._model_decoder_sigma
        pos_enc = self._pos_encoding(_unit(pts.reshape(-1, 3)))
        if self.enc_injection:
            sigma_feat = enc(pos_enc, ch, n)
        elif self.enc_concat:
            sigma_feat = enc(self._append_embedding(pos_enc, self.encoder_channel_embedding, ch, n, L, enc.dtype,
                                                    grouped))
        else:
            sigma_feat = enc(pos_enc)
        dec_in = F.relu(sigma_feat)
        if self.dec_injection:
            attn = dec(dec_in, ch, n)
        elif self.dec_concat:
            attn = dec(self._append_embedding(dec_in, self.decoder_channel_embedding, ch, n, L, dec.dtype, grouped))
        else:
            attn = dec(dec_in)
        if grouped:
            B, R, S = L
            dir_e = self._dir_encoding(_unit(_per_ray(view.reshape(-1, 3), L)))
            tx_e = self._tx_encoding(_unit(_per_pose(tx.reshape(-1, 3), L)))
            parts = [(sigma_feat, 1), (dir_e, S), (tx_e, R * S)]
            E = self.emb_dim_sig
            if self.sig_concat and E >= 8 and E % 8 == 0 and sum(p.size(1) for p, _ in parts) + E <= 512:
                base = grouped_concat(parts + [(self.signal_channel_embedding[ch], R * S)], N, sigma_feat.dtype,
                                      splits=[1, 1, R, R])
            else:
                base = grouped_concat(parts, N, sigma_feat.dtype, splits=[1, 1, R])
                if self.sig_concat:
                    base = torch.cat([base, _embed_rows(self.signal_channel_embedding, ch, n).to(base.dtype)], -1)
            return torch.abs(F.leaky_relu(attn)).view(bs, n, 1), base
        dir_enc = _grouped(self._dir_encoding, _unit(view.reshape(-1, 3)), L, "ray")
        tx_enc = _grouped(self._tx_encoding, _unit(tx.reshape(-1, 3)), L, "pose")
        dt = sigma_feat.dtype
        sf = sigma_feat if L is None else sigma_feat.view(*L, -1)
        base = _cat_features([sf, dir_enc.to(dt), tx_enc.to(dt)], L)
        if self.sig_concat:
            base = torch.cat([base, _embed_rows(self.signal_channel_embedding, ch, n).to(dt)], -1)
        attn = torch.abs(F.leaky_relu(attn)).view(bs, n, 1)
        return attn, base

    def _trunk_fused(self, pts, view, tx, L):
        B, R, S = L
        bs, n = pts.size(0), pts.size(1)
        pos_enc = self._pos_encoding.forward_level_major(pts.reshape(-1, 3), unit_map=True)
        dir_e = self._dir_encoding(_unit(_per_ray(view.reshape(-1, 3), L)))
        tx_e = self._tx_encoding(_unit(_per_pose(tx.reshape(-1, 3), L)))
        packed = self._sigma_pack.get(_sigma.MESHRIR, _sigma_params(self), self._model_encoder_sigma.dtype)
        attn, base = _sigma.sigma_fwd(_sigma.MESHRIR, packed, bs * n, [(pos_enc, 1)],
                                      [(dir_e, S), (tx_e, R * S)], 128, 0.01)
        return attn.view(bs, n, 1), base

    def _trunk_fused_h1(self, pts, view, tx, L):
        B, R, S = L
        bs, n = pts.size(0), pts.size(1)
        pos_enc = self._pos_encoding.forward_level_major(pts.reshape(-1, 3), unit_map=True)
        w1 = self._model_signal.layers[0].weight
        dt = self._model_encoder_sigma.dtype
        wd, wt = _bias_columns(w1, dt)
        bias = _ray_pose_bias(self._dir_encoding, self._tx_encoding, view, tx, wd, wt, L, dt)
        if bias is None:
            dir_e = self._dir_encoding(_unit(_per_ray(view.reshape(-1, 3), L)))
            tx_e = self._tx_encoding(_unit(_per_pose(tx.reshape(-1, 3), L)))
            bias = dir_e.to(dt).float() @ wd
            bias = (bias.view(B, R, -1) + (tx_e.to(dt).float() @ wt).view(B, 1, -1))
            bias = bias.reshape(B * R, -1).contiguous()
        params = _sigma_params(self) + [w1[:, :128]]
        packed = self._sigma_pack.get(_sigma.MESHRIR_H1, params, dt)
        attn, h1 = _sigma.sigma_fwd(_sigma.MESHRIR_H1, packed, bs * n, [(pos_enc, 1)], [], 512, 0.01,
                                    bias=bias, bias_div=S)
        return attn.view(bs, n, 1), h1

    def _signal_hidden(self, pts, view, tx, ch_idx, ray_layout):
        if (not self._has_embed and _fused_sigma_ok(self, pts, ray_layout, _sigma.MESHRIR)
                and self.options.fused_h1 and _sigma.h1_ok(self)):
            attn, h1 = self._trunk_fused_h1(pts, view, tx, ray_layout)
            return attn, self._model_signal.hidden_from(h1, 1)
        attn, base = self._trunk(pts, view, tx, ch_idx, ray_layout)
        if self.sig_injection:
            return attn, self._model_signal.hidden(base, self._channel(pts, ch_idx), pts.size(1))
        return attn, self._model_signal.hidden(base)

    def forward(self, pts, view, tx, ch_idx=None, ray_layout=None):
        attn, h = self._signal_hidden(pts, view, tx, ch_idx, ray_layout)
        signal = self._model_signal.last(h)
        return attn, signal.view(pts.size(0), pts.size(1), self.signal_output_dim)

    def forward_fused(self, pts, view, tx, ch_idx=None, ray_layout=None):
        attn, h = self._signal_hidden(pts, view, tx, ch_idx, ray_layout)
        return (attn, h.view(pts.size(0), pts.size(1), -1), self._model_signal.layers[-1].weight,
                self._model_signal.dtype)

    def finish_signal(self, h):
        return self._model_signal.last(h.reshape(-1, h.size(-1))).view(h.size(0), h.size(1), -1)


class AVRModel_complex(nn.Module):

    def __init__(self, cfg, mlp_dtype=torch.float32, enc_dtype=torch.float32, options=None):
        super().__init__()
        o = self.options = resolve(options)
        self.leaky_relu = cfg["leaky_relu"]
        self.signal_output_dim = int(cfg["signal_output_dim"])
        E = lambda key, seed: HashGridEncoding(3, cfg[key], dtype=enc_dtype, seed=seed, options=o)
        self._pos_encoding = E("pos_encoding_sigma", 11)
        self._pos_signal_encoding = E("pos_encoding_sig", 12)
        self._tx_pos_encoding = E("tx_pos_encoding_sigma", 13)
        self._tx_pos_signal_encoding = E("tx_pos_encoding_sig", 14)
        self._dir_encoding = E("dir_encoding_sig", 15)
        self._tx_dir_encoding = E("tx_dir_encoding_sig", 16)
        n_in = self._pos_encoding.n_output_dims + self._tx_pos_encoding.n_output_dims
        self._model_encoder_sigma = MLP(n_in, 256, cfg["sigma_encoder_network"], mlp_dtype, o)
        self._model_decoder_sigma = MLP(256, 1, cfg["sigma_decoder_network"], mlp_dtype, o)
        n_sig = (256 + self._dir_encoding.n_output_dims + self._tx_dir_encoding.n_output_dims
                 + self._pos_signal_encoding.n_output_dims + self._tx_pos_signal_encoding.n_output_dims)
        self._model_signal = MLP(n_sig, self.signal_output_dim, cfg["signal_network"], mlp_dtype, o)
        self._sigma_pack = _sigma.SigmaWeights()

    accepts_ray_layout = True
    supports_fused_head = True
    draws_no_device_rng = True

    def forward(self, pts, view, tx, tx_view, ray_layout=None):
        attn, base = self._trunk(pts, view, tx, tx_view, ray_layout)
        signal = self._model_signal(base)
        return attn, signal.reshape(pts.size(0), pts.size(1), self.signal_output_dim)

    def forward_fused(self, pts, view, tx, tx_view, ray_layout=None):
        attn, base = self._trunk(pts, view, tx, tx_view, ray_layout)
        link = [False]
        h = self._model_signal.hidden(base, link)
        if torch.is_grad_enabled() and len(self._model_signal.layers) > 1:
            self._relu_link = link
        return (attn, h.view(pts.size(0), pts.size(1), -1), self._model_signal.layers[-1].weight,
                self._model_signal.dtype)

    finish_signal = AVRModel.finish_signal

    def _trunk(self, pts, view, tx, tx_view, ray_layout):
        bs, n = pts.size(0), pts.size(1)
        L = ray_layout
        if _fused_sigma_ok(self, pts, L, _sigma.RAF):
            return self._trunk_fused(pts, view, tx, tx_view, L)
# ... 53 lines not shown
```

avr_amd/options.py:

```python
from __future__ import annotations

import dataclasses
import os

TUNING_ENV = ("AVR_NSPLIT", "AVR_KSPLIT")


@dataclasses.dataclass(frozen=True)
class KernelOptions:
    fused_sigma: bool = True
    fused_h1: bool = True
    grouped_concat: bool = True
    fused_dgrad: bool = True
    narrow: str = "80"
    out1: bool = True
    chembed: bool = True
    tunableop: bool = True
    wgrad_min: int = 512 * 512
    hashgrid_bwd: str = "partitioned"

    def __post_init__(self):
        if self.narrow not in ("80", "all", "off"):
            raise ValueError(f"KernelOptions.narrow must be '80', 'all' or 'off', not {self.narrow!r}")
        if self.hashgrid_bwd not in ("partitioned", "partitioned_add", "atomic"):
            raise ValueError("KernelOptions.hashgrid_bwd must be 'partitioned', 'partitioned_add' or 'atomic'")

    def replace(self, **kw) -> "KernelOptions":
        return dataclasses.replace(self, **kw)

    @classmethod
    def from_env(cls, base: "KernelOptions | None" = None) -> "KernelOptions":
        base = base or cls()
        kw = {}
        for f in dataclasses.fields(cls):
            v = os.environ.get("AVR_OPT_" + f.name.upper())
            if v is None:
                continue
            if f.type in ("bool", bool):
                kw[f.name] = v not in ("0", "false", "False", "")
            elif f.type in ("int", int):
                kw[f.name] = int(v)
            else:
                kw[f.name] = v
        return dataclasses.replace(base, **kw)


DEFAULT = KernelOptions()


def resolve(options) -> KernelOptions:
    if options is None:
        return DEFAULT
    if not isinstance(options, KernelOptions):
        raise TypeError("options must be an avr_amd.KernelOptions")
    return options


def tuning_env() -> tuple:
    return tuple(os.environ.get(k) for k in TUNING_ENV)


def apply(module, options: KernelOptions):
    options = resolve(options)
    for m in module.modules():
        if hasattr(m, "options"):
            m.options = options
    return module
```

avr_amd/renderer.py:

```python
from __future__ import annotations

import ctypes
import math
import threading

import torch
import torch.nn as nn

from . import _lib
from ._lib import DTYPE_BF16, DTYPE_F16, DTYPE_F32, _ptr, _stream, render_params
from .options import tuning_env
from .wcache import cache_lookup, cache_store, capturing, cast_weight


_RENDER_KEYS = ("n_samples", "near", "far", "n_azi", "n_ele", "speed", "fs", "pathloss",
                "xyz_min", "xyz_max")


class _NoGuard:
    def __enter__(self):
        return None

    def __exit__(self, *exc):
        return False


_NO_GUARD = _NoGuard()


def _on(dev):
    return _NO_GUARD if torch.cuda.current_device() == dev.index else torch.cuda.device(dev)


def _f32_on(t, dev):
    if t.device != dev or t.dtype != torch.float32:
        t = t.to(dev, torch.float32)
    return t if t.is_contiguous() else t.contiguous()


def _dtype_code(t):
    if t.dtype == torch.float32:
        return DTYPE_F32
    if t.dtype == torch.float16:
        return DTYPE_F16
    if t.dtype == torch.bfloat16:
        return DTYPE_BF16
    raise TypeError(f"unsupported dtype {t.dtype} (float32, float16 or bfloat16)")


class Tables:

    def __init__(self, p, device):
        S, T = p.n_samples, p.T
        F = T // 2 + 1
        f32 = dict(dtype=torch.float32, device=device)
        self.d_vals = torch.empty(S, **f32)
        self.frac = torch.empty(S, **f32)
        self.shift = torch.empty(S, dtype=torch.int32, device=device)
        self.pl = torch.empty(p.pl_len, **f32)
        self.phase = torch.empty(S, F, 2, **f32)
        self.twiddle = torch.empty(T, 2, **f32)
        n = 2 * (F - 1)
        self.ir_n = n
        self.ir_twiddle = torch.empty(max(n, 2), 2, **f32)
        st = _stream(device)
        with torch.cuda.device(device):
            _lib.call("avr_tables", ctypes_ref(p), _ptr(self.d_vals), _ptr(self.frac),
                      _ptr(self.shift), _ptr(self.pl), _ptr(self.phase), _ptr(self.twiddle), st)
            if n >= 2:
                _lib.call("avr_ir_twiddle", n, _ptr(self.ir_twiddle), st)
        shifts = self.shift.cpu()
        self.max_shift = int(shifts.max().item()) if S > 0 else 0
        self.ptrs = _lib.TablePtrs(self.d_vals.data_ptr(), self.shift.data_ptr(),
                                   self.pl.data_ptr(), self.phase.data_ptr(),
                                   self.twiddle.data_ptr(),
                                   self.ir_twiddle.data_ptr() if n >= 2 else None)
        self._layouts = {}

    def core_layout(self, p, B, sig_code):
        key = (p.n_rays, B, sig_code) + tuning_env()
        v = self._layouts.get(key)
        if v is None:
            with _TABLE_LOCK:
                v = self._layouts.get(key)
                if v is None:
                    off = (ctypes.c_int64 * 5)()
                    sp = (ctypes.c_int32 * 2)()
                    _lib.call("avr_render_core_layout", ctypes_ref(p), B, sig_code, off, sp)
                    v = (tuple(off), int(sp[0]), int(sp[1]))
                    self._layouts[key] = v
        return v


def ctypes_ref(p):
# ... 216 lines not shown
        R, S = p.n_rays, p.n_samples
        st = _stream(dev)
        gz = _grad_z(p, tables, grad_out.reshape(B * C, -1, 2), B * C, dev, st)
        grad_signal = torch.empty_like(signal)
        grad_w = torch.empty(B, R, S, dtype=torch.float32, device=dev)
        if C == 1:
            _lib.call("avr_ray_reduce_bwd", ctypes_ref(p), B, _ptr(signal), _dtype_code(signal),
                      _ptr(gz), _ptr(wg), _ptr(delay), _ptr(grad_signal), _ptr(grad_w), st)
            grad_w = grad_w * gain.reshape(-1, R, 1)
        else:
            _lib.call("avr_ray_reduce_mc_bwd", ctypes_ref(p), B, C, _ptr(signal), _dtype_code(signal),
                      _ptr(gz), _ptr(wg), _ptr(delay), _ptr(gain), _gain_stride(gain), _ptr(grad_signal),
                      _ptr(grad_w), st)
        grad_attn = _grad_attn(p, tables, attn, grad_w, st) if ctx.needs_input_grad[0] else None
        return (grad_attn, grad_signal if ctx.needs_input_grad[1] else None,
                None, None, None, None, None, None) + (None,) * ctx.n_opt


class SHDecode(torch.autograd.Function):

    @staticmethod
    def forward(ctx, amb, dec):
        B, K, F = amb.shape[:3]
        out = torch.empty(B, dec.size(0), F, 2, dtype=torch.float32, device=amb.device)
        _lib.call("avr_sh_decode_fwd", B, dec.size(0), K, F, _ptr(dec), _ptr(amb), _ptr(out), _stream(amb.device))
        ctx.save_for_backward(dec)
        return out

    @staticmethod
    def backward(ctx, grad_out):
        (dec,) = ctx.saved_tensors
        B, E, F = grad_out.shape[:3]
        grad_out = grad_out.contiguous()
        grad_amb = torch.empty(B, dec.size(1), F, 2, dtype=torch.float32, device=grad_out.device)
        _lib.call("avr_sh_decode_bwd", B, E, dec.size(1), F, _ptr(dec), _ptr(grad_out), _ptr(grad_amb),
                  _stream(grad_out.device))
        return grad_amb, None


def resolve_sh_decoder(sh_decoder, C, F, dev):
    d = torch.as_tensor(sh_decoder).detach()
    if d.is_complex():
        d = torch.view_as_real(d.to(torch.complex64))
    if d.dim() != 4 or d.size(-1) != 2 or d.size(0) < 1:
        raise ValueError(f"sh_decoder [E, K, F] complex or [E, K, F, 2] expected, got {tuple(d.shape)}")
    if d.size(1) != C or d.size(2) != F:
        raise ValueError(f"sh_decoder has K = {d.size(1)} channels and F = {d.size(2)} bins; the render has "
                         f"{C} and {F}")
    return _f32_on(d, dev)


def sh_decode(amb, dec):
    amb = amb.float().contiguous()
    with _on(amb.device):
        return SHDecode.apply(amb, resolve_sh_decoder(dec, amb.size(1), amb.size(2), amb.device))


def _packed_head_weight(w_master, W, cache, pref, shape_key, st):
    key = (W.data_ptr(), w_master._version, shape_key)
    cache = cache and not capturing()
    if cache:
        hit = cache_lookup(w_master, "_avr_headpack", key)
        if hit is not None:
            return hit
    B, K, code = shape_key[2], shape_key[3], shape_key[4]
    Wp = torch.empty_like(W)
    _lib.call("avr_head_pack_w", pref, B, K, _ptr(W), code, _ptr(Wp), st)
    return cache_store(w_master, "_avr_headpack", key, Wp) if cache else Wp


def _packed_exact_weight(w_master, W, cache, pref, shape_key, nbytes, st):
    key = (W.data_ptr(), w_master._version, shape_key)
    cache = cache and not capturing()
    if cache:
        hit = cache_lookup(w_master, "_avr_exactpack", key)
        if hit is not None:
            return hit
    K, code = shape_key[1], shape_key[2]
    Wf = torch.empty(nbytes // 2, dtype=W.dtype, device=W.device)
    _lib.call("avr_head_pack_w_exact", pref, K, _ptr(W), code, _ptr(Wf), st)
    return cache_store(w_master, "_avr_exactpack", key, Wf) if cache else Wf


class FusedHeadCore(torch.autograd.Function):

    @staticmethod
    def forward(ctx, attn, h, w_master, dtype, p, tables, rays_o, position_tx, dirs, cache=False, exact=False,
                relu_h=False, timer=None, gain=None):
        dev = h.device
        B, K = h.size(0), h.size(-1)
        S, T = p.n_samples, p.T
        st = _stream(dev)
        pref = ctypes_ref(p)
        W = cast_weight(w_master, dtype, cache)
        code = _dtype_code(h)
        w, delay = _weights(p, attn, rays_o, position_tx, dirs, tables, st)
        R = p.n_rays
        if gain is not None:
            w = w * gain.unsqueeze(-1)
        perm = torch.empty(B, S, R, dtype=torch.int32, device=dev)
        ws = torch.empty(B, S, R, dtype=torch.float32, device=dev)
        cnt = torch.empty(B, S, T, dtype=torch.int32, device=dev)
        _lib.call("avr_head_sort", pref, B, _ptr(w), _ptr(delay), _ptr(perm), _ptr(ws), _ptr(cnt), st)
        if exact:
            ns, wbytes = ctypes.c_int32(0), ctypes.c_int64(0)
            _lib.call("avr_head_exact_layout", pref, B, K, code, ctypes.byref(ns), ctypes.byref(wbytes))
            n_split = ns.value
            part = torch.empty(n_split, B, S, T, dtype=torch.float32, device=dev)
            queue = torch.empty(256, dtype=torch.int32, device=dev)
            Wf = _packed_exact_weight(w_master, W, cache, pref, (p.T, K, code), wbytes.value, st)
            ev0, ev1 = timer.head_events(delay, tables.shift, K) if timer is not None else (None, None)
            if ev0 is not None:
                ev0.record()
            _lib.call("avr_head_fwd_exact", pref, B, K, _ptr(h), _ptr(Wf), code, _ptr(perm), _ptr(ws), _ptr(cnt),
                      _ptr(delay), n_split, _ptr(part), _ptr(queue), st)
            if ev1 is not None:
                ev1.record()
        else:
            ns = ctypes.c_int32(0)
            _lib.call("avr_head_splits", pref, B, K, code, ctypes.byref(ns))
            n_split = ns.value
            part = torch.empty(n_split, B, S, T, dtype=torch.float32, device=dev)
            Wp = _packed_head_weight(w_master, W, cache, pref, (p.T, R, B, K, code), st)
            _lib.call("avr_head_fwd", pref, B, K, _ptr(h), _ptr(Wp), code, _ptr(perm), _ptr(ws), _ptr(cnt),
                      n_split, _ptr(part), st)
        out = _spectrum(p, tables, part, n_split, B, dev, st)
        ctx.p, ctx.tables, ctx.relu_h, ctx.gain = p, tables, relu_h, gain
        ctx.save_for_backward(attn, h, W, w, delay, perm, ws, cnt)
        return out

    @staticmethod
    def backward(ctx, grad_out):
        attn, h, W, w, delay, perm, ws, cnt = ctx.saved_tensors
        p, tables = ctx.p, ctx.tables
        dev = h.device
        B, K = h.size(0), h.size(-1)
        R, S, T = p.n_rays, p.n_samples, p.T
        st = _stream(dev)
        pref = ctypes_ref(p)
        code = _dtype_code(h)
        gz = _grad_z(p, tables, grad_out, B, dev, st)
        nbytes = ctypes.c_int64(0)
        _lib.call("avr_head_bwd_workspace", pref, B, K, code, ctypes.byref(nbytes))
        work = torch.empty(max(1, nbytes.value // 4), dtype=torch.float32, device=dev)
        grad_h = torch.empty_like(h)
        grad_w = torch.empty(B, R, S, dtype=torch.float32, device=dev)
        grad_W = torch.empty(T, K, dtype=torch.float32, device=dev)
        _lib.call("avr_head_bwd2", pref, B, K, _ptr(h), _ptr(W), code, _ptr(w), _ptr(delay), _ptr(perm),
                  _ptr(ws), _ptr(cnt), _ptr(gz), int(ctx.relu_h), _ptr(grad_h), _ptr(grad_w), _ptr(grad_W),
                  _ptr(work), nbytes.value, st)
        if ctx.gain is not None:
            grad_w = grad_w * ctx.gain.unsqueeze(-1)
        grad_attn = _grad_attn(p, tables, attn, grad_w, st) if ctx.needs_input_grad[0] else None
        return (grad_attn, grad_h if ctx.needs_input_grad[1] else None,
                grad_W if ctx.needs_input_grad[2] else None, None, None, None, None, None, None, None, None, None,
                None, None)


def _poison_nonfinite(out, tensors, ir_out=None):
    bad = None
    for t in tensors:
        b = ~torch.isfinite(t).all()
        bad = b if bad is None else bad | b
    poison = torch.where(bad, float("nan"), 0.0)
    if ir_out is not None:
        ir_out.add_(poison)
    return out + poison


def normalize_points(input_pts, xyz_min, xyz_max):
    return 2 * (input_pts - xyz_min) / (xyz_max - xyz_min) - 1


def denormalize_points(input_pts, xyz_min, xyz_max):
    return (input_pts + 1) / 2 * (xyz_max - xyz_min) + xyz_min


def draw_jitter(n_azi, n_ele):
    u_azi = torch.rand(n_azi)
    torch.rand(n_ele)
    return u_azi


def ray_directions(n_azi, n_ele, random_azi=True, device=None):
    device = torch.device("cuda", torch.cuda.current_device()) if device is None else device
    u = draw_jitter(n_azi, n_ele)
    if not random_azi:
        u = torch.zeros_like(u)
    p = render_params(dict(n_azi=n_azi, n_ele=n_ele, n_samples=1, far=1, near=0, xyz_min=-1,
                           xyz_max=1, fs=1, speed=1, pathloss=1), 2)
    dirs = torch.empty(n_azi * n_ele + 2, 3, dtype=torch.float32, device=device)
    u_dev = u.to(device, non_blocking=True)
    _lib.call("avr_ray_directions", ctypes_ref(p), _ptr(u_dev), _ptr(dirs), _stream(device))
    return dirs, None, None


class _SamplePoses(torch.autograd.Function):

    @staticmethod
    def forward(ctx, render, u_azi, rays_o, position_tx, direction_tx):
        poses = (rays_o, position_tx, direction_tx)
        pts, view, tx, dtx, geom = render._sample(
            *(None if t is None else t.detach() for t in poses), u_azi)
        ctx.k = 2.0 / render._params(2, geom["n_rays"]).span
        ctx.like = [None if t is None else (t.shape, t.dtype, t.device) for t in poses]
        need = ctx.needs_input_grad[2:]
        ctx.mark_non_differentiable(view, *(t for t, n in zip((pts, tx, dtx), need) if t is not None and not n))
        ctx.set_materialize_grads(False)
        return pts, tx, dtx, view, geom

    @staticmethod
    def backward(ctx, g_pts, g_tx, g_dtx, *_):
        def pose_grad(g, like, k, need):
            if g is None or like is None or not need:
                return None
            s = g.sum(dim=1, dtype=torch.float32)
            if k is not None:
                s = s * k
            shape, dtype, device = like
            return s.to(device=device, dtype=dtype).reshape(shape)

        need = ctx.needs_input_grad
        return (None, None, pose_grad(g_pts, ctx.like[0], ctx.k, need[2]),
                pose_grad(g_tx, ctx.like[1], ctx.k, need[3]), pose_grad(g_dtx, ctx.like[2], None, need[4]))


class AVRRender(nn.Module):

    def __init__(self, networks_fn, **kwargs) -> None:
        super().__init__()
        self.network_fn = networks_fn
        for k in _RENDER_KEYS:
            setattr(self, k, kwargs[k])
        self._cfg = {k: kwargs[k] for k in _RENDER_KEYS}
        self.ray_range = None
        self.fused_head = bool(kwargs.get("fused_head", True))
        self.propagate_nonfinite = bool(kwargs.get("propagate_nonfinite", False))
        self.exact_head = bool(kwargs.get("exact_head", True))
        self.head_relu_link = bool(kwargs.get("head_relu_link", True))
# ... 127 lines not shown
            attn = attn.to(dev)
        attn = attn.reshape(B, -1)
        if not attn.is_contiguous():
            attn = attn.contiguous()
        T = signal.size(-1)
        if signal.device != dev:
            signal = signal.to(dev)
        signal = signal.reshape(B, -1, T)
        if not signal.is_contiguous():
            signal = signal.contiguous()
        R = geom["n_rays"]
        if attn.size(1) != R * S or signal.size(1) != R * S:
            raise ValueError(f"network output has {signal.size(1)} ray-samples, expected "
                             f"{R}x{S}={R * S}")
        p = self._params(T, R)
        with _on(dev):
            tables = get_tables(p, dev)
            check_config(p, tables)
            if ray_gain is not None:
                gain, flat = resolve_ray_gain(ray_gain, geom)
                C, F = gain.size(-2), T // 2 + 1
                dec = None if sh_decoder is None else resolve_sh_decoder(sh_decoder, C, F, dev)
                args = (attn, signal, gain, p, tables, geom["rays_o"], geom["position_tx"], geom["dirs"])
                if not (torch.is_grad_enabled() and (attn.requires_grad or signal.requires_grad)):
                    out = _render_core_mc_fwd(*args, mc_reduce=self.mc_reduce)[0].view(B, C, F, 2)
                else:
                    out = RenderCoreMC.apply(*args, self.mc_reduce)
                if dec is not None:
                    out = SHDecode.apply(out, dec)
                if ir_out is not None:
                    _lib.call("avr_irfft", out.size(0) * out.size(1), F, _ptr(out), _ptr(tables.ir_twiddle),
                              _ptr(ir_out), _stream(dev))
                if self.propagate_nonfinite:
                    out = _poison_nonfinite(out, (attn, signal), ir_out)
                return out[:, 0] if flat and dec is None else out
            if not (torch.is_grad_enabled() and (attn.requires_grad or signal.requires_grad)):
                out = _render_core_fwd(attn, signal, p, tables, geom["rays_o"],
                                       geom["position_tx"], geom["dirs"], ir_out, self.kernel_timer)[0]
            else:
                out = RenderCore.apply(attn, signal, p, tables, geom["rays_o"], geom["position_tx"],
                                       geom["dirs"], ir_out, self.kernel_timer)
            if self.propagate_nonfinite:
                out = _poison_nonfinite(out, (attn, signal), ir_out)
            return out

    def _head_supported(self, geom, h, weight, dtype):
        if dtype not in (torch.float32, torch.bfloat16, torch.float16):
            return False
        p = self._params(weight.size(0), geom["n_rays"])
        code = {torch.bfloat16: DTYPE_BF16, torch.float16: DTYPE_F16}.get(dtype, DTYPE_F32)
        n = ctypes.c_int32(0)
        lib = _lib.load()
        if lib.avr_head_splits(ctypes_ref(p), geom["B"], h.size(-1), code, ctypes.byref(n)) != 0:
            return False
        if self._exact_for(dtype, h.size(-1)):
            nb = ctypes.c_int64(0)
            return lib.avr_head_exact_layout(ctypes_ref(p), geom["B"], h.size(-1), code, ctypes.byref(n),
                                             ctypes.byref(nb)) == 0
        return True

    def _exact_for(self, dtype, K):
        return self.exact_head and dtype in (torch.float16, torch.bfloat16) and K % 16 == 0 and K <= 512

    def render_from_hidden(self, attn, h, weight, dtype, geom, relu_link=None, gain=None):
        dev, B = geom["device"], geom["B"]
        S = int(self.n_samples)
        attn = attn.to(dev).reshape(B, -1)
        if attn.dtype not in (torch.float32, torch.float16, torch.bfloat16):
            attn = attn.float()
        attn = attn.contiguous()
        K, T = h.size(-1), weight.size(0)
        h = h.to(dev, dtype).reshape(B, -1, K).contiguous()
        R = geom["n_rays"]
        if attn.size(1) != R * S or h.size(1) != R * S:
            raise ValueError(f"network output has {h.size(1)} ray-samples, expected {R}x{S}={R * S}")
        p = self._params(T, R)
        with _on(dev):
            tables = get_tables(p, dev)
            check_config(p, tables)
            exact = self._exact_for(dtype, K)
            relu_h = relu_link is not None and torch.is_grad_enabled()
            out = FusedHeadCore.apply(attn, h, weight, dtype, p, tables, geom["rays_o"],
                                      geom["position_tx"], geom["dirs"], not torch.is_grad_enabled(), exact,
                                      relu_h, self.kernel_timer, gain)
            if relu_h:
                relu_link[0] = True
            if self.propagate_nonfinite:
                out = _poison_nonfinite(out, (attn, h, weight))
            return out

    def forward(self, rays_o, position_tx, direction_tx=None, ch_idx=None, *, ray_gain=None, sh_decoder=None,
                u_azi=None):
        return self._render(rays_o, position_tx, direction_tx, ch_idx, None, u_azi=u_azi, ray_gain=ray_gain,
                            sh_decoder=sh_decoder)

    def render_ir(self, rays_o, position_tx, direction_tx=None, ch_idx=None, *, ray_gain=None, sh_decoder=None,
                  u_azi=None):
        ir = []
        grad = torch.is_grad_enabled()
        out = self._render(rays_o, position_tx, direction_tx, ch_idx, None if grad else ir, u_azi=u_azi,
                           ray_gain=ray_gain, sh_decoder=sh_decoder)
        if ir:
            return out, ir[0]
        if out.dim() == 4:
            B, C, F = out.shape[:3]
            return out, spectrum_to_ir(out.reshape(B * C, F, 2)).view(B, C, -1)
        return out, spectrum_to_ir(out)

    def _render(self, rays_o, position_tx, direction_tx, ch_idx, ir_slot, u_azi=None, ray_gain=None,
                sh_decoder=None):
        if sh_decoder is not None and ray_gain is None:
            raise ValueError("sh_decoder needs ray_gain (the channels it decodes, e.g. spatial.ambisonic(3))")
        pts, view, tx, dtx, geom = self.sample(rays_o, position_tx, direction_tx, u_azi=u_azi)
        gain = flat = None
        ears = None if sh_decoder is None else int(torch.as_tensor(sh_decoder).size(0))
        if ray_gain is not None:
            if self.ray_range is not None:
                raise NotImplementedError("ray_gain with sharded rays")
            gain, flat = resolve_ray_gain(ray_gain, geom)
        kw = {} if ch_idx is None else {"ch_idx": ch_idx}
        if getattr(self.network_fn, "accepts_ray_layout", False):
            kw["ray_layout"] = (geom["B"], geom["n_rays"], int(self.n_samples))
        net_in = (pts, view, tx) if dtx is None else (pts, view, tx, dtx)
        if self.fused_head and getattr(self.network_fn, "supports_fused_head", False):
            attn, h, weight, dtype = self.network_fn.forward_fused(*net_in, **kw)
            if (gain is None or (gain.size(-2) == 1 and sh_decoder is None)) \
                    and self._head_supported(geom, h, weight, dtype):
                link = getattr(self.network_fn, "_relu_link", None) if self.head_relu_link else None
                self.network_fn.__dict__.pop("_relu_link", None)
                out = self.render_from_hidden(attn, h, weight, dtype, geom, link,
                                              None if gain is None else gain.squeeze(-2))
                return out if gain is None or flat else out.unsqueeze(1)
            signal = self.network_fn.finish_signal(h)
            if gain is None:
                return self.render_from_network_output(attn, signal, geom)
            return self.render_from_network_output(attn, signal, geom,
                                                   self._ir_out(signal, geom, gain, flat, ir_slot, ears),
                                                   ray_gain=gain[0] if flat else gain, sh_decoder=sh_decoder)
        if dtx is not None:
            attn, signal = self.network_fn(pts, view, tx, dtx, **kw)
        else:
            attn, signal = self.network_fn(pts, view, tx, **kw)
        ir_out = self._ir_out(signal, geom, gain, flat, ir_slot, ears)
        if gain is None:
            return self.render_from_network_output(attn, signal, geom, ir_out)
        return self.render_from_network_output(attn, signal, geom, ir_out, ray_gain=gain[0] if flat else gain,
                                               sh_decoder=sh_decoder)

    @staticmethod
    def _ir_out(signal, geom, gain, flat, ir_slot, ears=None):
        if ir_slot is None:
            return None
        F = signal.size(-1) // 2 + 1
        if F < 2:
            return None
        lead = (geom["B"],) if gain is None or flat else (geom["B"], gain.size(-2))
        if ears is not None:
            lead = (geom["B"], ears)
        ir_out = torch.empty(*lead, 2 * (F - 1), dtype=torch.float32, device=geom["device"])
        ir_slot.append(ir_out)
        return ir_out


class _IRFFT(torch.autograd.Function):

    @staticmethod
    def forward(ctx, out):
# ... 46 lines not shown
```

include/avr_hip.h:

```cpp
#ifndef AVR_HIP_H
#define AVR_HIP_H

#include <stdint.h>

#ifdef __cplusplus
extern "C" {
#endif

#define AVR_ABI_VERSION 2

#define AVR_DTYPE_F32 0
#define AVR_DTYPE_F16 1
#define AVR_DTYPE_BF16 2

#define AVR_E_ARG 1001
#define AVR_E_CONFIG 1002

typedef struct avr_render_params {
    int32_t n_azi;
    int32_t n_ele;
    int32_t n_samples;
    int32_t T;
    int32_t n_rays;
    float depth_scale;
// ... 62 lines not shown
                          const float* gain, int64_t gain_b_stride, int32_t n_split, float* part,
                          void* stream);

int avr_reduce_mc_splits(const avr_render_params* p, int32_t B, int32_t C, int32_t sig_dtype,
                         int32_t* n_split, int32_t* max_rays);

int avr_ray_reduce_mc16_fwd(const avr_render_params* p, int32_t B, int32_t C, const void* signal,
                            int32_t sig_dtype, const float* w, const int32_t* delay,
                            const float* gain, int64_t gain_b_stride, int32_t n_split, float* part,
                            void* stream);
int32_t avr_reduce_mc16_max_rays(void);

int avr_sh_decode_fwd(int32_t B, int32_t E, int32_t K, int32_t F, const float* dec, const float* amb,
                      float* out, void* stream);
int avr_sh_decode_bwd(int32_t B, int32_t E, int32_t K, int32_t F, const float* dec,
                      const float* grad_out, float* grad_amb, void* stream);

int avr_dft_phase_fwd(const avr_render_params* p, int32_t B, const float* part,
                      int32_t n_split, const float* pl_table, const int32_t* shift,
                      const float* phase, const float* twiddle, int32_t k_split,
                      float* spart, void* stream);

int avr_spectrum_finalize(int32_t B, int32_t P, int32_t F, const float* spart, float* out,
                          void* stream);

#define AVR_IRFFT_MAX_N 13476
int avr_irfft(int32_t B, int32_t F, const float* spec, const float* tw, float* ir,
              void* stream);
int avr_irfft_bwd(int32_t B, int32_t F, const float* grad_ir, const float* tw, float* grad_spec,
                  void* stream);

typedef struct avr_table_ptrs {
    const float* d_vals;
    const int32_t* shift;
    const float* pl_table;
    const float* phase;
    const float* twiddle;
    const float* ir_twiddle;
} avr_table_ptrs;

int avr_render_core_layout(const avr_render_params* p, int32_t B, int32_t sig_dtype,
                           int64_t* offsets, int32_t* splits);

int avr_render_core_fwd(const avr_render_params* p, int32_t B, const void* attn,
                        int32_t attn_dtype, const void* signal, int32_t sig_dtype,
                        const float* rays_o, const float* pos_tx, const float* dirs,
                        const avr_table_ptrs* tables, void* workspace, int64_t workspace_bytes,
                        float* out, float* ir, void* ev_begin, void* ev_end, void* stream);

int avr_dft_phase_bwd(const avr_render_params* p, int32_t B, const float* grad_out,
                      const float* pl_table, const int32_t* shift, const float* phase,
                      const float* twiddle, float* gz, void* stream);

int avr_ray_reduce_bwd(const avr_render_params* p, int32_t B, const void* signal,
                       int32_t sig_dtype, const float* gz, const float* w,
                       const int32_t* delay, void* grad_signal, float* grad_w, void* stream);

int avr_ray_reduce_mc_bwd(const avr_render_params* p, int32_t B, int32_t C, const void* signal,
                          int32_t sig_dtype, const float* gz, const float* w, const int32_t* delay,
                          const float* gain, int64_t gain_b_stride, void* grad_signal, float* grad_w,
                          void* stream);

int avr_weights_bwd(const avr_render_params* p, int32_t B, const void* attn, int32_t attn_dtype,
                    const float* d_vals, const float* grad_w, void* grad_attn, void* stream);

int avr_hashgrid_fwd(int64_t N, int32_t n_levels, const float* x, const void* params,
                     int32_t param_dtype, const int64_t* level_offset, const float* level_scale,
                     const int32_t* level_res, void* out, int32_t out_dtype, void* stream);

int avr_hashgrid_fwd_lm(int64_t N, int32_t n_levels, const float* x, const void* params,
                        int32_t param_dtype, const int64_t* level_offset, const float* level_scale,
                        const int32_t* level_res, void* out, int32_t out_dtype, void* stream);
int avr_hashgrid_fwd_lm_unit(int64_t N, int32_t n_levels, const float* x, const void* params,
                             int32_t param_dtype, const int64_t* level_offset, const float* level_scale,
                             const int32_t* level_res, void* out, int32_t out_dtype, void* stream);

int avr_ray_pose_bias(int32_t B, int32_t R, int32_t S, const float* view, const float* tx,
                      int32_t dir_levels, const void* dir_params, const int64_t* dir_offset,
                      const float* dir_scale, const int32_t* dir_res, int32_t tx_levels,
                      const void* tx_params, const int64_t* tx_offset, const float* tx_scale,
                      const int32_t* tx_res, int32_t param_dtype, int32_t enc_dtype,
                      int32_t mlp_dtype, const float* w_dir, const float* w_tx, int32_t n_out,
                      float* bias, void* stream);

int avr_hashgrid_bwd(int64_t N, int32_t n_levels, const float* x, const void* grad_out,
                     int32_t grad_dtype, const int64_t* level_offset, const float* level_scale,
                     const int32_t* level_res, float* grad_params, void* stream);

int avr_hashgrid_bwd_workspace(int64_t N, int32_t n_levels, const int64_t* level_offset, int64_t* bytes);
int avr_hashgrid_bwd_partitioned(int64_t N, int32_t n_levels, const float* x, const void* grad_out,
                                 int32_t grad_dtype, const int64_t* level_offset, const float* level_scale,
                                 const int32_t* level_res, float* grad_params, void* workspace,
                                 int64_t workspace_bytes, void* stream);
int avr_hashgrid_bwd_partitioned_set(int64_t N, int32_t n_levels, const float* x, const void* grad_out,
                                     int32_t grad_dtype, const int64_t* level_offset, const float* level_scale,
                                     const int32_t* level_res, float* grad_params, void* workspace,
                                     int64_t workspace_bytes, void* stream);

int avr_hashgrid_bwd_input_workspace(int64_t N, int32_t n_levels, int64_t* bytes);
int avr_hashgrid_bwd_input(int64_t N, int32_t n_levels, const float* x, const void* params,
                           int32_t param_dtype, const void* grad_out, int32_t grad_dtype,
                           const int64_t* level_offset, const float* level_scale,
                           const int32_t* level_res, float* grad_x, void* workspace,
                           int64_t workspace_bytes, void* stream);

int avr_linear_wgrad_splits(int64_t N, int32_t M, int32_t K, int32_t* splits);
int avr_narrow_mm(int64_t N, int32_t R, int32_t C, const void* X, const void* Bt, int32_t dtype, int32_t act,
                  const void* mask, void* Y, void* stream);
int avr_linear_out1_fwd(int64_t N, int32_t K, const void* x, const void* w, int32_t dtype, void* y, void* stream);
int avr_linear_out1_workspace(int32_t K, int64_t* floats);
int avr_linear_out1_bwd(int64_t N, int32_t K, const void* x, const void* w, const void* grad_y, int32_t dtype,
                        void* grad_x, float* workspace, float* grad_w, void* stream);
int avr_linear512_pack_w2(const void* W, int32_t dtype, int32_t transpose, void* Wf, void* stream);
int avr_linear512_mask_fwd(int64_t M, const void* x, const void* Wf, int32_t dtype, const void* mask, void* y,
                           void* stream);

#ifdef AVR_SHAPE_PROBES
int avr_linear512_pack_w(const void* W, int32_t dtype, void* Wf, void* stream);
int avr_linear512_relu_fwd(int64_t M, const void* x, const void* Wf, int32_t dtype, void* y, void* stream);
int avr_mlp512x2_pack_w(const void* W1, const void* W2, int32_t dtype, void* Wf, void* stream);
int avr_mlp512x2_fwd(int64_t M, const void* x, const void* Wf, int32_t dtype, void* y, void* stream);
#endif
int avr_linear_wgrad(int64_t N, int32_t M, int32_t K, const void* grad_y, const void* x,
                     float* workspace, int32_t splits, float* grad_w, void* stream);

#define AVR_SIGMA_MESHRIR 0
#define AVR_SIGMA_RAF 1
#define AVR_SIGMA_MESHRIR_H1 2
#define AVR_SIGMA_MAX_EXTRA 4
typedef struct {
    const void* data;
    int32_t dtype;
    int32_t rows_div;
    int64_t lm_rows;
} avr_feat_src;

typedef struct {
    int32_t variant;
    int32_t tile_cfg;
    int64_t n_samples;
    float leaky_slope;
    avr_feat_src input[2];
    int32_t n_extra;
    avr_feat_src extra[AVR_SIGMA_MAX_EXTRA];
    int32_t extra_width[AVR_SIGMA_MAX_EXTRA];
    const float* bias;
    int32_t bias_div;
    int32_t dtype;
} avr_sigma_desc;

int avr_sigma_pack_bytes(int32_t variant, int64_t* bytes);
int avr_sigma_desc_size(void);
int avr_sigma_fwd(const avr_sigma_desc* d, const void* wpack, void* base, int32_t ldb, void* attn,
                  void* stream);

#define AVR_CONCAT_MAX_SRC 8
typedef struct {
    const void* data;
    void* grad;
    int32_t dtype;
    int32_t rows_div;
    int32_t width;
    int32_t split;
} avr_concat_src;

int avr_concat_fwd(int64_t N, int32_t n_src, const avr_concat_src* src, void* out, int32_t out_dtype,
                   void* stream);
int avr_concat_bwd(int64_t N, int32_t n_src, const avr_concat_src* src, const void* grad_out,
                   int32_t grad_dtype, float* workspace, void* stream);

int avr_head_splits(const avr_render_params* p, int32_t B, int32_t K, int32_t dtype,
                    int32_t* n_split);
int avr_head_sort(const avr_render_params* p, int32_t B, const float* w, const int32_t* delay,
                  int32_t* perm, float* ws, int32_t* cnt, void* stream);
int avr_head_pack_w(const avr_render_params* p, int32_t B, int32_t K, const void* W, int32_t dtype,
                    void* Wp, void* stream);
int avr_head_fwd(const avr_render_params* p, int32_t B, int32_t K, const void* h, const void* W,
                 int32_t dtype, const int32_t* perm, const float* ws, const int32_t* cnt,
                 int32_t n_split, float* zpart, void* stream);
int avr_head_exact_layout(const avr_render_params* p, int32_t B, int32_t K, int32_t dtype,
                          int32_t* n_split, int64_t* wpack_bytes);
int avr_head_pack_w_exact(const avr_render_params* p, int32_t K, const void* W, int32_t dtype, void* Wf,
                          void* stream);
int avr_head_fwd_exact(const avr_render_params* p, int32_t B, int32_t K, const void* h, const void* Wf,
                       int32_t dtype, const int32_t* perm, const float* ws, const int32_t* cnt,
                       const int32_t* delay, int32_t n_split, float* zpart, int32_t* queue, void* stream);
int avr_head_bwd_workspace(const avr_render_params* p, int32_t B, int32_t K, int32_t dtype,
                           int64_t* bytes);
int avr_head_bwd(const avr_render_params* p, int32_t B, int32_t K, const void* h, const void* W,
                 int32_t dtype, const float* w, const int32_t* delay, const int32_t* perm,
                 const float* ws, const int32_t* cnt, const float* gz, void* grad_h,
                 float* grad_w, float* grad_W, float* workspace, int64_t workspace_bytes,
                 void* stream);
int avr_head_bwd2(const avr_render_params* p, int32_t B, int32_t K, const void* h, const void* W,
                  int32_t dtype, const float* w, const int32_t* delay, const int32_t* perm,
                  const float* ws, const int32_t* cnt, const float* gz, int32_t relu_mask, void* grad_h,
                  float* grad_w, float* grad_W, float* workspace, int64_t workspace_bytes, void* stream);

int avr_criterion_window_len(void);
int avr_criterion_workspace(int32_t B, int32_t F, int64_t* bytes);
int avr_criterion_fwd(int32_t B, int32_t F, const float* weights, const float* pred,
                      const float* ori, const float* wtab, const float* tw512, const float* irtw,
                      float* pred_time, float* ori_time, float* losses, void* workspace,
                      int64_t workspace_bytes, void* stream);
int avr_criterion_fwd2(int32_t B, int32_t F, const float* weights, const float* pred,
                       const float* ori, const float* wtab, const float* tw512, const float* irtw,
                       float* pred_time, float* ori_time, float* losses, float* total, void* workspace,
                       int64_t workspace_bytes, void* stream);
int avr_criterion_bwd(int32_t B, int32_t F, const float* weights, const float* pred,
                      const float* ori, const float* pred_time, const float* ori_time,
                      const float* grad_losses,
                      const float* grad_pred_time, const float* wtab, const float* tw512,
                      const float* irtw, void* workspace, int64_t workspace_bytes,
                      float* grad_pred, void* stream);

int avr_das_workspace(int64_t* bytes);
int avr_das_fwd(int32_t n, const float* pred_time, const float* ori_time, const float* steer,
                const float* angles, const float* tw512, float beta, float w_reg, float w_ce,
                float* losses, void* workspace, int64_t workspace_bytes, void* stream);
int avr_das_bwd(int32_t n, const float* steer, const float* angles, const float* tw512, float beta,
                float w_reg, float w_ce, const float* grad_losses, void* workspace,
                int64_t workspace_bytes, float* grad_pred_time, void* stream);

#define AVR_METRICS_COLS 9
int avr_metrics_workspace(int32_t B, int32_t n, int64_t* bytes);
int avr_metrics(int32_t B, int32_t n, double fs, int32_t s50, int32_t window, const float* ori,
                const float* pred, const float* ir_twiddle, const float* win_table,
                const float* tw512, float* rows, float* means, float* ori_energy,
                float* pred_energy, void* workspace, int64_t workspace_bytes, void* stream);

int avr_scale_sanitize(int32_t n_tensors, float* const* ptrs, const int64_t* sizes,
                       const float* coef, void* stream);
int avr_grad_clip_workspace(int32_t n_tensors, const int64_t* sizes, int64_t* bytes);
int avr_grad_clip_coef(int32_t n_tensors, const float* const* ptrs, const int64_t* sizes, float max_norm,
                       void* workspace, int64_t workspace_bytes, float* total, float* coef, void* stream);
int avr_adam_step(int32_t n_tensors, float* const* params, const float* const* grads,
                  float* const* exp_avg, float* const* exp_avg_sq, const int64_t* sizes,
                  const float* step_size, const float* bc2_sqrt, double beta1, double beta2,
                  float eps, float weight_decay, const float* coef, void* stream);

int avr_group_bias_relu_fwd(int64_t N, int32_t W, int64_t rows_per_group, int32_t C, const void* y,
                            int32_t dtype, const float* table, const int64_t* idx, void* out,
                            void* stream);
int avr_group_bias_relu_workspace(int64_t N, int32_t W, int64_t rows_per_group, int64_t* bytes);
int avr_group_bias_relu_bwd(int64_t N, int32_t W, int64_t rows_per_group, int32_t C, const void* gy,
                            const void* out, int32_t dtype, const int64_t* idx, void* g,
                            void* workspace, int64_t workspace_bytes, float* g_table, void* stream);

#define AVR_DTYPE_F64 3
int avr_conv_source(int32_t S, int32_t C, int32_t Nh, int64_t L, const float* h, const float* x,
                    float* y, void* stream);
int avr_conv_trajectory(int32_t P, int32_t C, int32_t Nh, int64_t L, int64_t hop, int64_t fade,
                        const float* h, const float* x, float* y, void* stream);
int avr_sosfiltfilt_workspace(int64_t rows, int64_t n, int32_t n_sections, int32_t padlen,
                              int64_t* bytes);
int avr_sosfiltfilt(int64_t rows, int64_t n, int32_t n_sections, int32_t padlen, const double* sos,
                    const double* zi, const void* y, int32_t in_dtype, void* out, int32_t out_dtype,
                    void* workspace, int64_t workspace_bytes, void* stream);

int avr_doa_das_workspace(int64_t G, int32_t nfft, int32_t K, int64_t* bytes);
int avr_doa_das(int64_t G, int32_t n, int32_t nfft, int32_t K, const float* pred_ir,
                const float* ori_ir, const float* steer, const float* angles, const double* tw,
                double beta, const void* position_rx, const void* position_tx, int32_t pos_dtype,
                double* out, void* workspace, int64_t workspace_bytes, void* stream);
int avr_doa_frames(int64_t G, int64_t n, int32_t L, int32_t H, int64_t n_frames, int32_t nfft,
                   int32_t hop, int32_t k_lo, int32_t K, int32_t algo, float floor, const void* y,
                   int32_t y_dtype, const float* tw, const float* win, const float* steer,
                   int32_t* est, uint8_t* valid, float* spectrum, void* stream);
int avr_doa_frame_stats(int64_t G, int64_t n_frames, const int32_t* est, const uint8_t* valid,
// ... 8 lines not shown
```

Baseline: 2.299 billion ray-samples/s.

## Co-launch hashgrid encoding with ray-pose bias and fold queue reset into sort

Adds a combined kernel that runs the level-major hashgrid forward and the ray/pose bias computation as extra grid rows of one launch, so the small bias kernel no longer runs serially after the grid encoding. Separately, the head sort kernel now zeroes the exact-head work queue, which removes the queue-clearing step from the exact head forward path by default. This saves kernel launches and lets the bias work fill idle CUs, at the cost of the bias part running at 256 threads instead of 512 and a more complex combined grid.

```diff
diff --git a/avr_amd/_lib.py b/avr_amd/_lib.py
--- a/avr_amd/_lib.py
+++ b/avr_amd/_lib.py
@@ -125,6 +125,10 @@
     "avr_ray_pose_bias": (ctypes.c_int, [_c_i32, _c_i32, _c_i32, _vp, _vp, _c_i32, _vp, _vp, _vp, _vp,
                                          _c_i32, _vp, _vp, _vp, _vp, _c_i32, _c_i32, _c_i32, _vp, _vp,
                                          _c_i32, _vp, _vp]),
+    "avr_hashgrid_fwd_lm_unit_bias": (ctypes.c_int, [_c_i64, _c_i32, _vp, _vp, _c_i32, _vp, _vp, _vp, _vp, _c_i32,
+                                                     _c_i32, _c_i32, _c_i32, _vp, _vp, _c_i32, _vp, _vp, _vp, _vp,
+                                                     _c_i32, _vp, _vp, _vp, _vp, _c_i32, _c_i32, _c_i32, _vp, _vp,
+                                                     _c_i32, _vp, _vp]),
     "avr_hashgrid_bwd": (ctypes.c_int, [_c_i64, _c_i32, _vp, _vp, _c_i32, _vp, _vp, _vp, _vp, _vp]),
     "avr_hashgrid_bwd_workspace": (ctypes.c_int, [_c_i64, _c_i32, _vp, _vp]),
     "avr_hashgrid_bwd_partitioned": (ctypes.c_int, [_c_i64, _c_i32, _vp, _vp, _c_i32, _vp, _vp, _vp, _vp, _vp,
@@ -144,11 +148,14 @@
     "avr_linear_out1_bwd": (ctypes.c_int, [_c_i64, _c_i32, _vp, _vp, _vp, _c_i32, _vp, _vp, _vp, _vp]),
     "avr_head_splits": (ctypes.c_int, [_vp, _c_i32, _c_i32, _c_i32, _vp]),
     "avr_head_sort": (ctypes.c_int, [_vp, _c_i32, _vp, _vp, _vp, _vp, _vp, _vp]),
+    "avr_head_sort_queue": (ctypes.c_int, [_vp, _c_i32, _vp, _vp, _vp, _vp, _vp, _vp, _vp]),
     "avr_head_pack_w": (ctypes.c_int, [_vp, _c_i32, _c_i32, _vp, _c_i32, _vp, _vp]),
     "avr_head_exact_layout": (ctypes.c_int, [_vp, _c_i32, _c_i32, _c_i32, _vp, _vp]),
     "avr_head_pack_w_exact": (ctypes.c_int, [_vp, _c_i32, _vp, _c_i32, _vp, _vp]),
     "avr_head_fwd_exact": (ctypes.c_int, [_vp, _c_i32, _c_i32, _vp, _vp, _c_i32, _vp, _vp, _vp, _vp, _c_i32,
                                           _vp, _vp, _vp]),
+    "avr_head_fwd_exact_queued": (ctypes.c_int, [_vp, _c_i32, _c_i32, _vp, _vp, _c_i32, _vp, _vp, _vp, _vp, _c_i32,
+                                                 _vp, _vp, _vp]),
     "avr_head_fwd": (ctypes.c_int, [_vp, _c_i32, _c_i32, _vp, _vp, _c_i32, _vp, _vp, _vp, _c_i32, _vp,
                                     _vp]),
     "avr_head_bwd_workspace": (ctypes.c_int, [_vp, _c_i32, _c_i32, _c_i32, _vp]),
diff --git a/avr_amd/csrc/common.h b/avr_amd/csrc/common.h
--- a/avr_amd/csrc/common.h
+++ b/avr_amd/csrc/common.h
@@ -35,6 +35,8 @@
                const float* tw512, void* ws, int64_t ws_bytes, float* out, void* stream);
 
 inline hipStream_t as_stream(void* s) { return reinterpret_cast<hipStream_t>(s); }
+
+constexpr int kExactQueueInts = 256;
 
 constexpr size_t kLdsDefault = 64 * 1024;
 
diff --git a/avr_amd/csrc/hashgrid.hip b/avr_amd/csrc/hashgrid.hip
--- a/avr_amd/csrc/hashgrid.hip
+++ b/avr_amd/csrc/hashgrid.hip
@@ -207,11 +207,9 @@
     }
 };
 
-template <typename Tp, typename To, bool ROW_MAJOR = false, bool GROUP = false>
-__global__ __launch_bounds__(256) void hashgrid_fwd_lm_kernel(int64_t N, const float* __restrict__ x,
-                                                              const Tp* __restrict__ params,
-                                                              LevelTable lt, To* __restrict__ out, int unit) {
-    const int l = blockIdx.y;
+template <typename Tp, typename To, bool ROW_MAJOR, bool GROUP>
+__device__ __forceinline__ void fwd_lm_block(int64_t N, const float* __restrict__ x, const Tp* __restrict__ params,
+                                             const LevelTable& lt, To* __restrict__ out, int unit, int l, int L) {
     const int64_t i = (int64_t)blockIdx.x * 256 + threadIdx.x;
     if (i >= N) return;
     float xi[3] = {x[i * 3 + 0], x[i * 3 + 1], x[i * 3 + 2]};
@@ -250,7 +248,14 @@
 #pragma unroll
         for (int k = 0; k < 8; ++k) acc.add(wgt[k], CornerAcc<Tp>::load(table, ent[k]));
     }
-    store_pair(out, ROW_MAJOR ? i * (int64_t)gridDim.y + l : (int64_t)l * N + i, acc.get());
+    store_pair(out, ROW_MAJOR ? i * (int64_t)L + l : (int64_t)l * N + i, acc.get());
+}
+
+template <typename Tp, typename To, bool ROW_MAJOR = false, bool GROUP = false>
+__global__ __launch_bounds__(256) void hashgrid_fwd_lm_kernel(int64_t N, const float* __restrict__ x,
+                                                              const Tp* __restrict__ params,
+                                                              LevelTable lt, To* __restrict__ out, int unit) {
+    fwd_lm_block<Tp, To, ROW_MAJOR, GROUP>(N, x, params, lt, out, unit, blockIdx.y, gridDim.y);
 }
 
 template <typename Tp, typename Tg>
@@ -997,49 +1002,76 @@
 constexpr int kBias2Rays = 4;
 constexpr int kBias2Threads = 512;
 
+template <typename Tp, int NT>
+__device__ __forceinline__ void bias2_block(int64_t blk, int R, int S, const float* __restrict__ view,
+                                            const float* __restrict__ tx, const Tp* __restrict__ dp,
+                                            const LevelTable& dl, int dL, const Tp* __restrict__ tp,
+                                            const LevelTable& tl, int tL, int f16, int mlp_f16,
+                                            const float* __restrict__ wd, const float* __restrict__ wt, int nout,
+                                            float* __restrict__ bias) {
+    __shared__ float ed[kBias2Rays][2 * kMaxLevels];
+    __shared__ float et[2 * kMaxLevels];
+    const int64_t g0 = blk * kBias2Rays;
+    const int64_t b = g0 / R;
+    for (int q = threadIdx.x; q < (kBias2Rays + 1) * kMaxLevels; q += NT) {
+        const int j = q / kMaxLevels, l = q % kMaxLevels;
+        const bool is_tx = j == kBias2Rays;
+        if (l >= (is_tx ? tL : dL)) continue;
+        bias_features(is_tx, b, (g0 + j) % R, R, S, view, tx, dp, dl, tp, tl, l, f16, mlp_f16, is_tx ? et : ed[j]);
+    }
+    __syncthreads();
+    for (int o = threadIdx.x; o < nout; o += NT) {
+        constexpr int KB = 16;
+        float st = 0.0f;
+        for (int k0 = 0; k0 < 2 * tL; k0 += KB) {
+            float w[KB];
+#pragma unroll
+            for (int u = 0; u < KB; ++u) w[u] = k0 + u < 2 * tL ? wt[(int64_t)(k0 + u) * nout + o] : 0.0f;
+#pragma unroll
+            for (int u = 0; u < KB; ++u)
+                if (k0 + u < 2 * tL) st = fmaf(et[k0 + u], w[u], st);
+        }
+        float sd[kBias2Rays];
+#pragma unroll
+        for (int r = 0; r < kBias2Rays; ++r) sd[r] = 0.0f;
+        for (int k0 = 0; k0 < 2 * dL; k0 += KB) {
+            float w[KB];
+#pragma unroll
+            for (int u = 0; u < KB; ++u) w[u] = k0 + u < 2 * dL ? wd[(int64_t)(k0 + u) * nout + o] : 0.0f;
+#pragma unroll
+            for (int u = 0; u < KB; ++u)
+                if (k0 + u < 2 * dL)
+#pragma unroll
+                    for (int r = 0; r < kBias2Rays; ++r) sd[r] = fmaf(ed[r][k0 + u], w[u], sd[r]);
+        }
+#pragma unroll
+        for (int r = 0; r < kBias2Rays; ++r) bias[(g0 + r) * nout + o] = sd[r] + st;
+    }
+}
+
 template <typename Tp>
 __global__ __launch_bounds__(kBias2Threads) void ray_pose_bias2_kernel(
     int B, int R, int S, const float* __restrict__ view, const float* __restrict__ tx, const Tp* __restrict__ dp,
     LevelTable dl, int dL, const Tp* __restrict__ tp, LevelTable tl, int tL, int f16, int mlp_f16,
     const float* __restrict__ wd, const float* __restrict__ wt, int nout, float* __restrict__ bias) {
-    __shared__ float ed[kBias2Rays][2 * kMaxLevels];
-    __shared__ float et[2 * kMaxLevels];
-    const int64_t g0 = (int64_t)blockIdx.x * kBias2Rays;
-    const int64_t b = g0 / R;
-    for (int q = threadIdx.x; q < (kBias2Rays + 1) * kMaxLevels; q += kBias2Threads) {
-        const int j = q / kMaxLevels, l = q % kMaxLevels;
-        const bool is_tx = j == kBias2Rays;
-        if (l >= (is_tx ? tL : dL)) continue;
-        bias_features(is_tx, b, (g0 + j) % R, R, S, view, tx, dp, dl, tp, tl, l, f16, mlp_f16, is_tx ? et : ed[j]);
-    }
-    __syncthreads();
-    for (int o = threadIdx.x; o < nout; o += kBias2Threads) {
-        constexpr int KB = 16;
-        float st = 0.0f;
-        for (int k0 = 0; k0 < 2 * tL; k0 += KB) {
-            float w[KB];
-#pragma unroll
-            for (int u = 0; u < KB; ++u) w[u] = k0 + u < 2 * tL ? wt[(int64_t)(k0 + u) * nout + o] : 0.0f;
-#pragma unroll
-            for (int u = 0; u < KB; ++u)
-                if (k0 + u < 2 * tL) st = fmaf(et[k0 + u], w[u], st);
-        }
-        float sd[kBias2Rays];
-#pragma unroll
-        for (int r = 0; r < kBias2Rays; ++r) sd[r] = 0.0f;
-        for (int k0 = 0; k0 < 2 * dL; k0 += KB) {
-            float w[KB];
-#pragma unroll
-            for (int u = 0; u < KB; ++u) w[u] = k0 + u < 2 * dL ? wd[(int64_t)(k0 + u) * nout + o] : 0.0f;
-#pragma unroll
-            for (int u = 0; u < KB; ++u)
-                if (k0 + u < 2 * dL)
-#pragma unroll
-                    for (int r = 0; r < kBias2Rays; ++r) sd[r] = fmaf(ed[r][k0 + u], w[u], sd[r]);
-        }
-#pragma unroll
-        for (int r = 0; r < kBias2Rays; ++r) bias[(g0 + r) * nout + o] = sd[r] + st;
-    }
+    bias2_block<Tp, kBias2Threads>(blockIdx.x, R, S, view, tx, dp, dl, dL, tp, tl, tL, f16, mlp_f16, wd, wt, nout,
+                                   bias);
+}
+
+template <typename Tp, typename To, bool GROUP>
+__global__ __launch_bounds__(256) void hashgrid_fwd_lm_bias_kernel(
+    int64_t N, const float* __restrict__ x, const Tp* __restrict__ params, LevelTable lt, To* __restrict__ out,
+    int unit, int L, int64_t nbias, int R, int S, const float* __restrict__ view, const float* __restrict__ tx,
+    const Tp* __restrict__ dp, LevelTable dl, int dL, const Tp* __restrict__ tp, LevelTable tl, int tL, int f16,
+    int mlp_f16, const float* __restrict__ wd, const float* __restrict__ wt, int nout, float* __restrict__ bias) {
+    const int rows = (int)gridDim.y - L;
+    if ((int)blockIdx.y >= rows) {
+        fwd_lm_block<Tp, To, false, GROUP>(N, x, params, lt, out, unit, (int)blockIdx.y - rows, L);
+        return;
+    }
+    const int64_t blk = (int64_t)blockIdx.y * gridDim.x + blockIdx.x;
+    if (blk >= nbias) return;
+    bias2_block<Tp, 256>(blk, R, S, view, tx, dp, dl, dL, tp, tl, tL, f16, mlp_f16, wd, wt, nout, bias);
 }
 
 }
@@ -1074,6 +1106,47 @@
         };
         if (v2) return go(ray_pose_bias2_kernel<Tp>, dim3((unsigned)(rays / kBias2Rays)), dim3(kBias2Threads));
         return go(ray_pose_bias_kernel<Tp>, grid, dim3(256));
+    });
+}
+
+extern "C" int avr_hashgrid_fwd_lm_unit_bias(
+    int64_t N, int32_t n_levels, const float* x, const void* params, int32_t param_dtype,
+    const int64_t* level_offset, const float* level_scale, const int32_t* level_res, void* out, int32_t out_dtype,
+    int32_t B, int32_t R, int32_t S, const float* view, const float* tx, int32_t dir_levels, const void* dir_params,
+    const int64_t* dir_offset, const float* dir_scale, const int32_t* dir_res, int32_t tx_levels,
+    const void* tx_params, const int64_t* tx_offset, const float* tx_scale, const int32_t* tx_res,
+    int32_t bias_param_dtype, int32_t enc_dtype, int32_t mlp_dtype, const float* w_dir, const float* w_tx,
+    int32_t n_out, float* bias, void* stream) {
+    const char* what = "avr_hashgrid_fwd_lm_unit_bias";
+    LevelTable lt, dl, tl;
+    if (int e = fwd_prologue(what, N, n_levels, x, params, level_offset, level_scale, level_res, out, &lt)) return e;
+    AVR_REQUIRE(N >= 1 && B >= 1 && R >= 1 && S >= 1 && view && tx && dir_params && tx_params && w_dir && w_tx &&
+                    bias && n_out >= 1,
+                "avr_hashgrid_fwd_lm_unit_bias: bad args");
+    AVR_REQUIRE(enc_dtype == AVR_DTYPE_F16 || enc_dtype == AVR_DTYPE_F32, "avr_hashgrid_fwd_lm_unit_bias: enc dtype");
+    AVR_REQUIRE(mlp_dtype == AVR_DTYPE_BF16 || mlp_dtype == AVR_DTYPE_F16,
+                "avr_hashgrid_fwd_lm_unit_bias: mlp dtype");
+    if (R % kBias2Rays != 0 || bias_param_dtype != param_dtype)
+        return fail(AVR_E_CONFIG, "avr_hashgrid_fwd_lm_unit_bias: needs R % 4 == 0 and one table dtype");
+    if (int e = make_table(dir_levels, dir_offset, dir_scale, dir_res, &dl)) return e;
+    if (int e = make_table(tx_levels, tx_offset, tx_scale, tx_res, &tl)) return e;
+    const int64_t gx = (N + 255) / 256;
+    const int64_t nbias = (int64_t)B * R / kBias2Rays;
+    const int64_t rows = (nbias + gx - 1) / gx;
+    AVR_REQUIRE(n_levels + rows <= 65535, "avr_hashgrid_fwd_lm_unit_bias: too many rays for this many points");
+    const dim3 grid((unsigned)gx, (unsigned)(n_levels + rows));
+    const int f16 = enc_dtype == AVR_DTYPE_F16, mlp_f16 = mlp_dtype == AVR_DTYPE_F16;
+    const bool grp = ((uintptr_t)params & 15) == 0;
+    hipStream_t st = as_stream(stream);
+    return dispatch_fwd_dtypes(param_dtype, out_dtype, what, [&](auto pt, auto ot) {
+        using Tp = typename decltype(pt)::type;
+        using To = typename decltype(ot)::type;
+        auto kern = hashgrid_fwd_lm_bias_kernel<Tp, To, false>;
+        if constexpr (std::is_same_v<Tp, __half>)
+            if (grp) kern = hashgrid_fwd_lm_bias_kernel<Tp, To, true>;
+        return launch(what, kern, grid, dim3(256), 0, st, N, x, (const Tp*)params, lt, (To*)out, 1, (int)n_levels,
+                      nbias, (int)R, (int)S, view, tx, (const Tp*)dir_params, dl, (int)dir_levels,
+                      (const Tp*)tx_params, tl, (int)tx_levels, f16, mlp_f16, w_dir, w_tx, (int)n_out, bias);
     });
 }
 
diff --git a/avr_amd/csrc/head.hip b/avr_amd/csrc/head.hip
--- a/avr_amd/csrc/head.hip
+++ b/avr_amd/csrc/head.hip
@@ -426,10 +426,13 @@
                                                              const int32_t* __restrict__ delay,
                                                              int* __restrict__ perm_out,
                                                              float* __restrict__ ws_out,
-                                                             int* __restrict__ cnt_out) {
+                                                             int* __restrict__ cnt_out,
+                                                             int* __restrict__ queue) {
     extern __shared__ float lds_f[];
     const int T = pp.T, S = pp.n_samples;
     const int s = blockIdx.x, b = blockIdx.y;
+    if (queue != nullptr && s == 0 && b == 0)
+        for (int i = threadIdx.x; i < kExactQueueInts; i += kThreads) queue[i] = 0;
     const int nk = pow2_ceil(R);
     int* cnt = reinterpret_cast<int*>(lds_f);
     float* wr = reinterpret_cast<float*>(cnt + T);
@@ -1001,8 +1004,8 @@
     return 0;
 }
 
-extern "C" int avr_head_sort(const avr_render_params* p, int32_t B, const float* w, const int32_t* delay,
-                             int32_t* perm, float* ws, int32_t* cnt, void* stream) {
+extern "C" int avr_head_sort_queue(const avr_render_params* p, int32_t B, const float* w, const int32_t* delay,
+                                   int32_t* perm, float* ws, int32_t* cnt, int32_t* queue, void* stream) {
     AVR_REQUIRE(p && B >= 1 && w && delay && perm && ws && cnt, "avr_head_sort: bad args");
     const int R = n_rays(*p);
     HeadShape hs;
@@ -1010,7 +1013,13 @@
     hipStream_t st = as_stream(stream);
     const dim3 grid(p->n_samples, B);
     auto kern = hs.rpt == 4 ? head_sort_kernel<4> : hs.rpt == 8 ? head_sort_kernel<8> : head_sort_kernel<16>;
-    return launch("avr_head_sort", kern, grid, dim3(kThreads), hs.lds_sort, st, *p, R, w, delay, perm, ws, cnt);
+    return launch("avr_head_sort", kern, grid, dim3(kThreads), hs.lds_sort, st, *p, R, w, delay, perm, ws, cnt,
+                  (int*)queue);
+}
+
+extern "C" int avr_head_sort(const avr_render_params* p, int32_t B, const float* w, const int32_t* delay,
+                             int32_t* perm, float* ws, int32_t* cnt, void* stream) {
+    return avr_head_sort_queue(p, B, w, delay, perm, ws, cnt, nullptr, stream);
 }
 
 extern "C" int avr_head_fwd(const avr_render_params* p, int32_t B, int32_t K, const void* h,
diff --git a/avr_amd/csrc/head_exact.hip b/avr_amd/csrc/head_exact.hip
--- a/avr_amd/csrc/head_exact.hip
+++ b/avr_amd/csrc/head_exact.hip
@@ -328,8 +328,6 @@
     }
 }
 
-constexpr int kExactQueueInts = 256;
-
 int exact_ksm(int K) { return K <= 128 ? 8 : (K <= 256 ? 16 : 32); }
 
 struct ExactShape {
@@ -398,10 +396,10 @@
                   as_stream(stream), T, (int)K, KSM, (const uint16_t*)W, (frag8*)Wf, n);
 }
 
-extern "C" int avr_head_fwd_exact(const avr_render_params* p, int32_t B, int32_t K, const void* h, const void* Wf,
-                                  int32_t dtype, const int32_t* perm, const float* ws, const int32_t* cnt,
-                                  const int32_t* delay, int32_t n_split, float* zpart, int32_t* queue,
-                                  void* stream) {
+static int head_fwd_exact(const avr_render_params* p, int32_t B, int32_t K, const void* h, const void* Wf,
+                          int32_t dtype, const int32_t* perm, const float* ws, const int32_t* cnt,
+                          const int32_t* delay, int32_t n_split, float* zpart, int32_t* queue, void* stream,
+                          bool fill_queue) {
     AVR_REQUIRE(p && B >= 1 && h && Wf && perm && ws && cnt && delay && zpart && queue,
                 "avr_head_fwd_exact: bad args");
     if (int e = exact_check(p, K, dtype)) return e;
@@ -429,7 +427,7 @@
                 per_cu = 1;
             const int64_t gq = std::min<int64_t>((int64_t)device_cus() * per_cu / 8, (items + 7) / 8);
             const int grid = 8 * (int)std::max<int64_t>(gq, 1);
-            (void)hipMemsetAsync(queue, 0, kExactQueueInts * sizeof(int32_t), st);
+            if (fill_queue) (void)hipMemsetAsync(queue, 0, kExactQueueInts * sizeof(int32_t), st);
             return launch("avr_head_fwd_exact", kern, dim3(grid), dim3(64 * waves), lds, st, *p, (int)B, R, (int)K,
                           (const E*)hv, (const frag8*)Wf, perm, ws, cnt, delay, zpart, (int*)queue, (int)items, prio);
         };
@@ -447,3 +445,17 @@
         return go(head_exact_kernel<E, 32, 8, 256, 4, 1, false>, 32, 8, 256, 4, 1, h);
     });
 }
+
+extern "C" int avr_head_fwd_exact(const avr_render_params* p, int32_t B, int32_t K, const void* h, const void* Wf,
+                                  int32_t dtype, const int32_t* perm, const float* ws, const int32_t* cnt,
+                                  const int32_t* delay, int32_t n_split, float* zpart, int32_t* queue,
+                                  void* stream) {
+    return head_fwd_exact(p, B, K, h, Wf, dtype, perm, ws, cnt, delay, n_split, zpart, queue, stream, true);
+}
+
+extern "C" int avr_head_fwd_exact_queued(const avr_render_params* p, int32_t B, int32_t K, const void* h,
+                                         const void* Wf, int32_t dtype, const int32_t* perm, const float* ws,
+                                         const int32_t* cnt, const int32_t* delay, int32_t n_split, float* zpart,
+                                         int32_t* queue, void* stream) {
+    return head_fwd_exact(p, B, K, h, Wf, dtype, perm, ws, cnt, delay, n_split, zpart, queue, stream, false);
+}
diff --git a/avr_amd/model.py b/avr_amd/model.py
--- a/avr_amd/model.py
+++ b/avr_amd/model.py
@@ -481,6 +481,16 @@
 
 
 def _ray_pose_bias(dir_enc, tx_enc, view, tx, wd, wt, layout, mlp_dtype=torch.bfloat16):
+    args = _bias_call(dir_enc, tx_enc, view, tx, wd, wt, layout, mlp_dtype)
+    if args is None:
+        return None
+    from . import _lib
+    *call, bias, _keep = args
+    _lib.call("avr_ray_pose_bias", *call, bias.data_ptr(), torch.cuda.current_stream(view.device).cuda_stream)
+    return bias
+
+
+def _bias_call(dir_enc, tx_enc, view, tx, wd, wt, layout, mlp_dtype):
     B, R, S = layout
     if not (view.is_cuda and dir_enc.dtype == tx_enc.dtype and dir_enc.param_dtype == tx_enc.param_dtype
             and dir_enc.n_levels <= 32 and tx_enc.n_levels <= 32
@@ -493,13 +503,31 @@
     cache = not torch.is_grad_enabled()
     dtab, ttab = dir_enc.table(cache), tx_enc.table(cache)
     bias = torch.empty(B * R, wd.size(1), dtype=torch.float32, device=view.device)
-    st = torch.cuda.current_stream(view.device).cuda_stream
-    _lib.call("avr_ray_pose_bias", B, R, S, v.data_ptr(), t.data_ptr(),
-              dir_enc.n_levels, dtab.data_ptr(), *dir_enc.level_meta(),
-              tx_enc.n_levels, ttab.data_ptr(), *tx_enc.level_meta(), _code(dtab.dtype), _code(dir_enc.dtype),
-              _lib.DTYPE_F16 if mlp_dtype == torch.float16 else _lib.DTYPE_BF16,
-              wd.data_ptr(), wt.data_ptr(), wd.size(1), bias.data_ptr(), st)
-    return bias
+    return (B, R, S, v.data_ptr(), t.data_ptr(),
+            dir_enc.n_levels, dtab.data_ptr(), *dir_enc.level_meta(),
+            tx_enc.n_levels, ttab.data_ptr(), *tx_enc.level_meta(), _code(dtab.dtype), _code(dir_enc.dtype),
+            _lib.DTYPE_F16 if mlp_dtype == torch.float16 else _lib.DTYPE_BF16,
+            wd.data_ptr(), wt.data_ptr(), wd.size(1), bias, (v, t, dtab, ttab))
+
+
+def _grid_and_bias(pos_enc, pts, dir_enc, tx_enc, view, tx, wd, wt, layout, mlp_dtype):
+    B, R, S = layout
+    if R % 4 or pos_enc.param_dtype != dir_enc.param_dtype:
+        return None
+    args = _bias_call(dir_enc, tx_enc, view, tx, wd, wt, layout, mlp_dtype)
+    if args is None:
+        return None
+    from . import _lib
+    from .encoding import _code
+    *call, bias, _keep = args
+    x = pts.reshape(-1, 3).float().contiguous()
+    N = x.size(0)
+    out = torch.empty(pos_enc.n_levels, N, 2, dtype=pos_enc.dtype, device=x.device)
+    table = pos_enc.table(not torch.is_grad_enabled())
+    _lib.call("avr_hashgrid_fwd_lm_unit_bias", N, pos_enc.n_levels, x.data_ptr(), table.data_ptr(),
+              _code(table.dtype), *pos_enc.level_meta(), out.data_ptr(), _code(out.dtype), *call, bias.data_ptr(),
+              torch.cuda.current_stream(x.device).cuda_stream)
+    return out, bias
 
 
 def _sigma_params(model):
@@ -650,11 +678,18 @@
     def _trunk_fused_h1(self, pts, view, tx, L):
         B, R, S = L
         bs, n = pts.size(0), pts.size(1)
-        pos_enc = self._pos_encoding.forward_level_major(pts.reshape(-1, 3), unit_map=True)
         w1 = self._model_signal.layers[0].weight
         dt = self._model_encoder_sigma.dtype
         wd, wt = _bias_columns(w1, dt)
-        bias = _ray_pose_bias(self._dir_encoding, self._tx_encoding, view, tx, wd, wt, L, dt)
+        both = None
+        if self.options.bias_colaunch:
+            both = _grid_and_bias(self._pos_encoding, pts, self._dir_encoding, self._tx_encoding, view, tx, wd, wt,
+                                  L, dt)
+        if both is not None:
+            pos_enc, bias = both
+        else:
+            pos_enc = self._pos_encoding.forward_level_major(pts.reshape(-1, 3), unit_map=True)
+            bias = _ray_pose_bias(self._dir_encoding, self._tx_encoding, view, tx, wd, wt, L, dt)
         if bias is None:
             dir_e = self._dir_encoding(_unit(_per_ray(view.reshape(-1, 3), L)))
             tx_e = self._tx_encoding(_unit(_per_pose(tx.reshape(-1, 3), L)))
diff --git a/avr_amd/options.py b/avr_amd/options.py
--- a/avr_amd/options.py
+++ b/avr_amd/options.py
@@ -18,6 +18,8 @@
     tunableop: bool = True
     wgrad_min: int = 512 * 512
     hashgrid_bwd: str = "partitioned"
+    head_queue_fill: bool = False
+    bias_colaunch: bool = True
 
     def __post_init__(self):
         if self.narrow not in ("80", "all", "off"):
diff --git a/avr_amd/renderer.py b/avr_amd/renderer.py
--- a/avr_amd/renderer.py
+++ b/avr_amd/renderer.py
@@ -9,7 +9,7 @@
 
 from . import _lib
 from ._lib import DTYPE_BF16, DTYPE_F16, DTYPE_F32, _ptr, _stream, render_params
-from .options import tuning_env
+from .options import DEFAULT, KernelOptions, tuning_env
 from .wcache import cache_lookup, cache_store, capturing, cast_weight
 
 
@@ -392,11 +392,16 @@
     return cache_store(w_master, "_avr_exactpack", key, Wf) if cache else Wf
 
 
+def _network_options(network_fn):
+    o = getattr(network_fn, "options", None)
+    return o if isinstance(o, KernelOptions) else DEFAULT
+
+
 class FusedHeadCore(torch.autograd.Function):
 
     @staticmethod
     def forward(ctx, attn, h, w_master, dtype, p, tables, rays_o, position_tx, dirs, cache=False, exact=False,
-                relu_h=False, timer=None, gain=None):
+                relu_h=False, timer=None, gain=None, queue_fill=False):
         dev = h.device
         B, K = h.size(0), h.size(-1)
         S, T = p.n_samples, p.T
@@ -411,19 +416,21 @@
         perm = torch.empty(B, S, R, dtype=torch.int32, device=dev)
         ws = torch.empty(B, S, R, dtype=torch.float32, device=dev)
         cnt = torch.empty(B, S, T, dtype=torch.int32, device=dev)
-        _lib.call("avr_head_sort", pref, B, _ptr(w), _ptr(delay), _ptr(perm), _ptr(ws), _ptr(cnt), st)
+        queue = torch.empty(256, dtype=torch.int32, device=dev) if exact else None
+        _lib.call("avr_head_sort_queue", pref, B, _ptr(w), _ptr(delay), _ptr(perm), _ptr(ws), _ptr(cnt),
+                  None if queue_fill else _ptr(queue), st)
         if exact:
             ns, wbytes = ctypes.c_int32(0), ctypes.c_int64(0)
             _lib.call("avr_head_exact_layout", pref, B, K, code, ctypes.byref(ns), ctypes.byref(wbytes))
             n_split = ns.value
             part = torch.empty(n_split, B, S, T, dtype=torch.float32, device=dev)
-            queue = torch.empty(256, dtype=torch.int32, device=dev)
             Wf = _packed_exact_weight(w_master, W, cache, pref, (p.T, K, code), wbytes.value, st)
             ev0, ev1 = timer.head_events(delay, tables.shift, K) if timer is not None else (None, None)
             if ev0 is not None:
                 ev0.record()
-            _lib.call("avr_head_fwd_exact", pref, B, K, _ptr(h), _ptr(Wf), code, _ptr(perm), _ptr(ws), _ptr(cnt),
-                      _ptr(delay), n_split, _ptr(part), _ptr(queue), st)
+            _lib.call("avr_head_fwd_exact" if queue_fill else "avr_head_fwd_exact_queued", pref, B, K, _ptr(h),
+                      _ptr(Wf), code, _ptr(perm), _ptr(ws), _ptr(cnt), _ptr(delay), n_split, _ptr(part),
+                      _ptr(queue), st)
             if ev1 is not None:
                 ev1.record()
         else:
@@ -464,7 +471,7 @@
         grad_attn = _grad_attn(p, tables, attn, grad_w, st) if ctx.needs_input_grad[0] else None
         return (grad_attn, grad_h if ctx.needs_input_grad[1] else None,
                 grad_W if ctx.needs_input_grad[2] else None, None, None, None, None, None, None, None, None, None,
-                None, None)
+                None, None, None)
 
 
 def _poison_nonfinite(out, tensors, ir_out=None):
@@ -758,7 +765,8 @@
             relu_h = relu_link is not None and torch.is_grad_enabled()
             out = FusedHeadCore.apply(attn, h, weight, dtype, p, tables, geom["rays_o"],
                                       geom["position_tx"], geom["dirs"], not torch.is_grad_enabled(), exact,
-                                      relu_h, self.kernel_timer, gain)
+                                      relu_h, self.kernel_timer, gain,
+                                      _network_options(self.network_fn).head_queue_fill)
             if relu_h:
                 relu_link[0] = True
             if self.propagate_nonfinite:
diff --git a/include/avr_hip.h b/include/avr_hip.h
--- a/include/avr_hip.h
+++ b/include/avr_hip.h
@@ -168,6 +168,16 @@
                       const int32_t* tx_res, int32_t param_dtype, int32_t enc_dtype,
                       int32_t mlp_dtype, const float* w_dir, const float* w_tx, int32_t n_out,
                       float* bias, void* stream);
+int avr_hashgrid_fwd_lm_unit_bias(int64_t N, int32_t n_levels, const float* x, const void* params,
+                                  int32_t param_dtype, const int64_t* level_offset, const float* level_scale,
+                                  const int32_t* level_res, void* out, int32_t out_dtype, int32_t B, int32_t R,
+                                  int32_t S, const float* view, const float* tx, int32_t dir_levels,
+                                  const void* dir_params, const int64_t* dir_offset, const float* dir_scale,
+                                  const int32_t* dir_res, int32_t tx_levels, const void* tx_params,
+                                  const int64_t* tx_offset, const float* tx_scale, const int32_t* tx_res,
+                                  int32_t bias_param_dtype, int32_t enc_dtype, int32_t mlp_dtype,
+                                  const float* w_dir, const float* w_tx, int32_t n_out, float* bias,
+                                  void* stream);
 
 int avr_hashgrid_bwd(int64_t N, int32_t n_levels, const float* x, const void* grad_out,
                      int32_t grad_dtype, const int64_t* level_offset, const float* level_scale,
@@ -259,6 +269,8 @@
                     int32_t* n_split);
 int avr_head_sort(const avr_render_params* p, int32_t B, const float* w, const int32_t* delay,
                   int32_t* perm, float* ws, int32_t* cnt, void* stream);
+int avr_head_sort_queue(const avr_render_params* p, int32_t B, const float* w, const int32_t* delay,
+                        int32_t* perm, float* ws, int32_t* cnt, int32_t* queue, void* stream);
 int avr_head_pack_w(const avr_render_params* p, int32_t B, int32_t K, const void* W, int32_t dtype,
                     void* Wp, void* stream);
 int avr_head_fwd(const avr_render_params* p, int32_t B, int32_t K, const void* h, const void* W,
@@ -271,6 +283,10 @@
 int avr_head_fwd_exact(const avr_render_params* p, int32_t B, int32_t K, const void* h, const void* Wf,
                        int32_t dtype, const int32_t* perm, const float* ws, const int32_t* cnt,
                        const int32_t* delay, int32_t n_split, float* zpart, int32_t* queue, void* stream);
+int avr_head_fwd_exact_queued(const avr_render_params* p, int32_t B, int32_t K, const void* h, const void* Wf,
+                              int32_t dtype, const int32_t* perm, const float* ws, const int32_t* cnt,
+                              const int32_t* delay, int32_t n_split, float* zpart, int32_t* queue,
+                              void* stream);
 int avr_head_bwd_workspace(const avr_render_params* p, int32_t B, int32_t K, int32_t dtype,
                            int64_t* bytes);
 int avr_head_bwd(const avr_render_params* p, int32_t B, int32_t K, const void* h, const void* W,
```

New measurement: 2.299 billion ray-samples/s, median of 2. About the same (+0.0%).
